# EryiXie/PlaneRecNet

Hardware: AMD Instinct MI355X
Metric: img/s fwd+bwd @480×640 ResNet101-DCN, 1/2/4/8 MI355X + roofline % (higher is better)
Workload: dtype f32 (tensors and accumulation fp32; plain GEMMs and the tap-walked 4x4/s2, 1x1/s2 and sub-pixel convolutions >= 300 tiles: 2xfp16-piece split MFMA, fp32 accumulate; fp32-only rate in fp32_only_run)

## Files before the change

### include/prn.h

```cpp
#ifndef PRN_H
#define PRN_H
#include <stdint.h>
#ifdef __cplusplus
extern "C" {
#endif

#define PRN_BN_SPLITS 32

int prn_version(void);
const char* prn_last_error(void);

enum { PRN_IN_ZERO = 0, PRN_IN_REFLECT = 1, PRN_IN_UP2_REFLECT = 2, PRN_IN_DILATED = 3, PRN_IN_UP2_PHASE = 4,
       PRN_IN_EMBED1 = 5  };
enum { PRN_EPI_NONE = 0, PRN_EPI_RELU = 1, PRN_EPI_SIGMOID = 2 };

enum { PRN_SPLIT_OFF = 0, PRN_SPLIT_PLAN = 1, PRN_SPLIT_ALWAYS = 2 };
enum { PRN_PIECES_BF16 = 0, PRN_PIECES_F16 = 16 };
typedef struct prn_gemm_opts {
  int32_t split_mode;
  int32_t split_kind;
  int32_t split_products;
  int32_t split_min_tiles;
  float split_min_gflop;
  int32_t wgrad_wgs;
  int32_t wgrad_target;
  int32_t wgrad_split;
} prn_gemm_opts;
void prn_gemm_opts_default(prn_gemm_opts* o);

typedef struct prn_conv_desc {
  int32_t B, C, H, W;
  int32_t M;
  int32_t KH, KW;
  int32_t stride, pad;
  int32_t Ho, Wo;
  int32_t in_mode;
  int32_t dil;
  int32_t epilogue;
  int32_t ystride;
  int32_t yH, yW;
  int32_t reserved;
  prn_gemm_opts opts;
} prn_conv_desc;

int64_t prn_conv2d_fwd_ws_bytes(const prn_conv_desc* d);
int prn_conv2d_kernel_kind(const prn_conv_desc* d);
int prn_conv2d_fwd_partials(const prn_conv_desc* d, int64_t* offset_bytes);
int prn_gemm_pipe(int M, int K, int B, int HW, int nz, const prn_gemm_opts* opts);
int64_t prn_split_images_bytes(int M, int K, int nz);
int prn_split_prepare(const float* w, void* images, int M, int K, int nz, int kind, void* stream);
int prn_split_prepare_batched(const void* items_dev, int n_items, int64_t total_blocks, int64_t total_row_blocks, int kind, void* stream);
int prn_conv2d_fwd(const prn_conv_desc* d, const float* x, const float* w, const float* bias,
                   const float* addend, float* y, void* ws, void* stream);
#define PRN_TILE_COUNTERS 4096
int prn_conv2d_fwd_counted(const prn_conv_desc* d, const float* x, const float* w, const void* w_images, const float* bias, const float* addend, float* y,
                           void* ws, unsigned* counters, void* stream, int phase);
#define PRN_MAX_SEGMENTS 6
typedef struct prn_ragged {
  int32_t nseg;
  int32_t H[PRN_MAX_SEGMENTS], W[PRN_MAX_SEGMENTS];
} prn_ragged;
int prn_conv2d_fwd_ragged(const prn_conv_desc* d, const prn_ragged* rg, const float* x, const float* w, const float* bias,
                          const float* addend, float* y, void* stream);
int64_t prn_conv2d_wgrad_ragged_ws_bytes(const prn_conv_desc* d, const prn_ragged* rg);
int prn_conv2d_wgrad_ragged(const prn_conv_desc* d, const prn_ragged* rg, const float* x, const float* dy, float* dw, void* ws,
                            void* stream);

int prn_conv2d_fwd_phase(const prn_conv_desc* d, const float* x, const float* w, const float* bias,
                         const float* addend, float* y, void* ws, void* stream, int phase);

int prn_weight_flip_transpose(const float* w, float* wt, int M, int C, int KH, int KW, void* stream);

typedef struct prn_flip_item {
  const float* src;
  float* dst;
  int M, C, KH, KW;
  int64_t first;
} prn_flip_item;
int prn_weight_flip_transpose_batched(const prn_flip_item* items_dev, int n_items, int64_t total_blocks, void* stream);

int64_t prn_winograd_tiles(int B, int H, int W);
typedef struct prn_winograd_item {
  const float* src;
  float* u;
  float* ut;
  int M, C;
  int64_t first;
} prn_winograd_item;
int prn_winograd_weights_batched(const prn_winograd_item* items_dev, int n_items, int64_t total_blocks, void* stream);
int prn_winograd_input(const float* x, float* V, int B, int C, int H, int W, int in_mode, void* stream);
int64_t prn_gemm_batched_ws_bytes(int M, int C, int P, int nb, const prn_gemm_opts* opts);
int prn_gemm_batched(int M, int C, int P, int nb, const float* U, const void* u_images, const float* V, float* Y, void* ws, const prn_gemm_opts* opts,
                     void* stream);
int prn_winograd_output(const float* Y, const float* bias, const float* addend, float* y, int B, int M, int H, int W, int epilogue, void* stream);
int prn_winograd_output_bn_fwd(const float* Yt, float* x_out, float* stats, const float* gamma, const float* beta, float* y, float* running_mean,
                               float* running_var, int B, int M, int H, int W, float eps, float momentum, int relu, void* stream);
int prn_winograd_output_bn_bwd(const float* Yt, const float* x, const float* stats, const float* gamma, const float* beta, float* dx, float* dgamma,
                               float* dbeta, int B, int M, int H, int W, int relu, void* stream);
int64_t prn_winograd_wgrad_ws_bytes(int B, int C, int H, int W, int M, const prn_gemm_opts* opts);
int prn_winograd_dy(const float* dy, float* Y, int B, int M, int H, int W, void* stream);
int prn_gemm_batched_nt_splits(int M, int C, int P, int nb, const prn_gemm_opts* opts);
int prn_gemm_batched_nt_kind(int M, int C, int P, int nb, const prn_gemm_opts* opts);
int prn_gemm_batched_nt(int M, int C, int P, int nb, const float* A, const float* Bm, float* ws, const prn_gemm_opts* opts, void* stream);
int prn_winograd_dw(const float* partials, float* dw, int M, int C, int splits, void* stream);
int prn_conv3x3_winograd_wgrad(const float* x, const float* dy, float* dw, void* ws, int B, int C, int H, int W, int M, int in_mode, const prn_gemm_opts* opts,
                               void* stream, int phase);
int prn_conv3x3_winograd_wgrad_v(const float* V, const float* dy, float* dw, void* ws, int B, int C, int H, int W, int M, const prn_gemm_opts* opts, void* stream);
int64_t prn_winograd_tiles_ragged(const prn_ragged* rg, int B);
int64_t prn_conv3x3_winograd_ragged_ws_bytes(const prn_ragged* rg, int B, int C, int M, const prn_gemm_opts* opts);
int prn_conv3x3_winograd_ragged(const float* x, const float* U, const void* u_images, const float* bias, const float* addend, float* y, void* ws,
                                const prn_ragged* rg, int B, int C, int M, int epilogue, const prn_gemm_opts* opts, void* stream);
int64_t prn_winograd_wgrad_ragged_ws_bytes(const prn_ragged* rg, int B, int C, int M, const prn_gemm_opts* opts);
int prn_conv3x3_winograd_wgrad_ragged(const float* x, const float* dy, float* dw, void* ws, const prn_ragged* rg, int B, int C, int M, const prn_gemm_opts* opts,
                                      void* stream);
int64_t prn_conv3x3_winograd_ws_bytes(int B, int C, int H, int W, int M, const prn_gemm_opts* opts);
int prn_conv3x3_winograd(const float* x, const float* U, const void* u_images, const float* bias, const float* addend, float* y, void* ws, int B, int C, int H,
                         int W, int M, int in_mode, int epilogue, const prn_gemm_opts* opts, void* stream);

int64_t prn_conv2d_wgrad_ws_bytes(const prn_conv_desc* d);
int prn_conv2d_wgrad_kernel_kind(const prn_conv_desc* d, int G);
int prn_conv2d_wgrad(const prn_conv_desc* d, const float* x, const float* dy, float* dw, void* ws, void* stream);
#define PRN_WGRAD_GROUP_MAX 16
int64_t prn_conv2d_wgrad_grouped_ws_bytes(const prn_conv_desc* d, int G);
int prn_conv2d_wgrad_grouped(const prn_conv_desc* d, int G, const float* const* x, const float* const* dy, float* dw, void* ws, void* stream);
int prn_conv2d_wgrad_phase(const prn_conv_desc* d, const float* x, const float* dy, float* dw, void* ws, void* stream, int phase);

int prn_up2_phase_weights(const float* w, float* wp, int M, int C, void* stream);
int prn_up2_dgrad_weights(const float* w, float* kd, int M, int C, void* stream);
int prn_replicate_fold(const float* dp, float* dx, int B, int C, int H, int W, void* stream);
int prn_space_to_depth2(const float* in, float* out, int B, int C, int H, int W, void* stream);
int prn_up2_wgrad_combine(const float* dwp, float* dw, int M, int C, void* stream);

int prn_pad_fold(const float* dp, float* dx, int B, int C, int H, int W, int up2, void* stream);
// ... 233 lines not shown
```

### planerecnet_amd/_lib.py

```python
import ctypes
import os

_HERE = os.path.dirname(os.path.abspath(__file__))
LIB_PATH = os.environ.get("PRN_LIB") or os.path.join(_HERE, "libprn_hip.so")

c_int, c_float, c_void_p, c_i64 = ctypes.c_int, ctypes.c_float, ctypes.c_void_p, ctypes.c_int64


class GemmOpts(ctypes.Structure):
    _fields_ = [("split_mode", ctypes.c_int32), ("split_kind", ctypes.c_int32), ("split_products", ctypes.c_int32), ("split_min_tiles", ctypes.c_int32),
                ("split_min_gflop", ctypes.c_float), ("wgrad_wgs", ctypes.c_int32), ("wgrad_target", ctypes.c_int32), ("wgrad_split", ctypes.c_int32)]

    def key(self):
        return (self.split_mode, self.split_kind, self.split_products, self.split_min_tiles, self.split_min_gflop, self.wgrad_wgs, self.wgrad_target, self.wgrad_split)


SPLIT_OFF, SPLIT_PLAN, SPLIT_ALWAYS = 0, 1, 2
PIECES_BF16, PIECES_F16 = 0, 16


class ConvDesc(ctypes.Structure):
    _fields_ = [(n, ctypes.c_int32) for n in
                ("B", "C", "H", "W", "M", "KH", "KW", "stride", "pad", "Ho", "Wo", "in_mode", "dil", "epilogue", "ystride", "yH", "yW", "reserved")] + [
                    ("opts", GemmOpts)]


class Ragged(ctypes.Structure):
    _fields_ = [("nseg", ctypes.c_int32), ("H", ctypes.c_int32 * 6), ("W", ctypes.c_int32 * 6)]


class DcnDesc(ctypes.Structure):
    _fields_ = [(n, ctypes.c_int32) for n in ("B", "C", "H", "W", "M", "stride", "pad", "Ho", "Wo", "raw")] + [("max_offset", ctypes.c_float),
                                                                                                              ("epilogue", ctypes.c_int32),
                                                                                                              ("opts", GemmOpts)]


class BottleneckDesc(ctypes.Structure):
    _fields_ = [(n, ctypes.c_int32) for n in ("B", "C", "H", "W", "planes", "stride", "dcn", "downsample", "flags")] + [
        ("eps", ctypes.c_float * 4), ("momentum", ctypes.c_float * 4), ("max_offset", ctypes.c_float), ("reserved", ctypes.c_int32), ("opts", GemmOpts)]


class BottleneckParams(ctypes.Structure):
    _fields_ = [(n, ctypes.c_void_p) for n in (
        "w1", "w2", "w3", "wd", "b2", "w1_img", "w3_img", "wd_img", "u2", "u2_img", "w1_t", "w2_t", "w3_t", "wd_t", "w1_t_img", "w3_t_img", "wd_t_img", "ut2", "ut2_img",
        "w27", "b27", "w27_t", "w2_cols_t", "w2_cols_t_img")] + [(n, ctypes.c_void_p * 4) for n in ("gamma", "beta", "running_mean", "running_var")]


IN_ZERO, IN_REFLECT, IN_UP2_REFLECT, IN_DILATED, IN_UP2_PHASE, IN_EMBED1 = 0, 1, 2, 3, 4, 5
EPI_NONE, EPI_RELU, EPI_SIGMOID = 0, 1, 2
BN_SPLITS = 32

P = c_void_p
_DP = ctypes.POINTER(ConvDesc)
_OP = ctypes.POINTER(GemmOpts)
SIGNATURES = {
    "prn_version": (c_int, []),
    "prn_last_error": (ctypes.c_char_p, []),
    "prn_conv2d_fwd_ws_bytes": (c_i64, [_DP]),
    "prn_conv2d_kernel_kind": (c_int, [_DP]),
    "prn_conv2d_fwd_partials": (c_int, [_DP, ctypes.POINTER(c_i64)]),
    "prn_gemm_opts_default": (None, [_OP]),
    "prn_gemm_pipe": (c_int, [c_int, c_int, c_int, c_int, c_int, _OP]),
    "prn_split_images_bytes": (c_i64, [c_int, c_int, c_int]),
    "prn_split_prepare": (c_int, [P, P, c_int, c_int, c_int, c_int, P]),
    "prn_split_prepare_batched": (c_int, [P, c_int, c_i64, c_i64, c_int, P]),
    "prn_conv2d_fwd": (c_int, [_DP, P, P, P, P, P, P, P]),
    "prn_conv2d_fwd_ragged": (c_int, [_DP, P, P, P, P, P, P, P]),
    "prn_conv2d_wgrad_ragged_ws_bytes": (c_i64, [_DP, P]),
    "prn_conv2d_wgrad_ragged": (c_int, [_DP, P, P, P, P, P, P]),
    "prn_gn_relu_fwd_ragged": (c_int, [P, P, P, P, P, c_int, c_int, c_int, P, c_int, c_float, P]),
    "prn_gn_relu_bwd_ragged": (c_int, [P, P, P, P, P, P, P, P, c_int, c_int, c_int, P, c_int, P]),
    "prn_conv2d_fwd_phase": (c_int, [_DP, P, P, P, P, P, P, P, c_int]),
    "prn_conv2d_fwd_counted": (c_int, [_DP, P, P, P, P, P, P, P, P, P, c_int]),
    "prn_conv2d_wgrad_phase": (c_int, [_DP, P, P, P, P, P, c_int]),
    "prn_weight_flip_transpose": (c_int, [P, P, c_int, c_int, c_int, c_int, P]),
    "prn_weight_flip_transpose_batched": (c_int, [P, c_int, c_i64, P]),
    "prn_winograd_tiles": (c_i64, [c_int, c_int, c_int]),
    "prn_winograd_weights_batched": (c_int, [P, c_int, c_i64, P]),
    "prn_winograd_input": (c_int, [P, P, c_int, c_int, c_int, c_int, c_int, P]),
    "prn_gemm_batched_ws_bytes": (c_i64, [c_int, c_int, c_int, c_int, _OP]),
    "prn_gemm_batched": (c_int, [c_int, c_int, c_int, c_int, P, P, P, P, P, _OP, P]),
    "prn_winograd_output": (c_int, [P, P, P, P, c_int, c_int, c_int, c_int, c_int, P]),
    "prn_winograd_output_bn_fwd": (c_int, [P] * 8 + [c_int] * 4 + [c_float, c_float, c_int, P]),
    "prn_winograd_output_bn_bwd": (c_int, [P] * 8 + [c_int] * 5 + [P]),
    "prn_winograd_wgrad_ws_bytes": (c_i64, [c_int] * 5 + [_OP]),
    "prn_winograd_dy": (c_int, [P, P, c_int, c_int, c_int, c_int, P]),
    "prn_gemm_batched_nt_splits": (c_int, [c_int] * 4 + [_OP]),
    "prn_gemm_batched_nt_kind": (c_int, [c_int] * 4 + [_OP]),
    "prn_conv2d_wgrad_kernel_kind": (c_int, [_DP, c_int]),
    "prn_gemm_batched_nt": (c_int, [c_int, c_int, c_int, c_int, P, P, P, _OP, P]),
    "prn_winograd_dw": (c_int, [P, P, c_int, c_int, c_int, P]),
    "prn_conv3x3_winograd_wgrad": (c_int, [P, P, P, P, c_int, c_int, c_int, c_int, c_int, c_int, _OP, P, c_int]),
    "prn_winograd_tiles_ragged": (c_i64, [P, c_int]),
    "prn_conv3x3_winograd_ragged_ws_bytes": (c_i64, [P, c_int, c_int, c_int, _OP]),
    "prn_conv3x3_winograd_ragged": (c_int, [P, P, P, P, P, P, P, P, c_int, c_int, c_int, c_int, _OP, P]),
    "prn_winograd_wgrad_ragged_ws_bytes": (c_i64, [P, c_int, c_int, c_int, _OP]),
    "prn_conv3x3_winograd_wgrad_ragged": (c_int, [P, P, P, P, P, c_int, c_int, c_int, _OP, P]),
    "prn_conv3x3_winograd_wgrad_v": (c_int, [P, P, P, P, c_int, c_int, c_int, c_int, c_int, _OP, P]),
    "prn_conv3x3_winograd_ws_bytes": (c_i64, [c_int] * 5 + [_OP]),
    "prn_conv3x3_winograd": (c_int, [P, P, P, P, P, P, P, c_int, c_int, c_int, c_int, c_int, c_int, c_int, _OP, P]),
    "prn_conv2d_wgrad_ws_bytes": (c_i64, [_DP]),
    "prn_conv2d_wgrad_grouped_ws_bytes": (c_i64, [_DP, c_int]),
    "prn_conv2d_wgrad_grouped": (c_int, [_DP, c_int, P, P, P, P, P]),
    "prn_conv2d_wgrad": (c_int, [_DP, P, P, P, P, P]),
    "prn_pad_fold": (c_int, [P, P, c_int, c_int, c_int, c_int, c_int, P]),
    "prn_pad_fold_pitched": (c_int, [P, P, c_int, c_int, c_int, c_int, c_int, P]),
    "prn_up2_phase_weights": (c_int, [P, P, c_int, c_int, P]),
    "prn_up2_dgrad_weights": (c_int, [P, P, c_int, c_int, P]),
    "prn_up2_wgrad_combine": (c_int, [P, P, c_int, c_int, P]),
    "prn_space_to_depth2": (c_int, [P, P, c_int, c_int, c_int, c_int, P]),
    "prn_replicate_fold": (c_int, [P, P, c_int, c_int, c_int, c_int, P]),
    "prn_channel_sum": (c_int, [P, P, P, c_int, c_int, c_int, P]),
    "prn_dcn_sample": (c_int, [P, P, P] + [c_int] * 7 + [c_float, P]),
    "prn_dcn_sample_bwd_ws_bytes": (c_i64, [c_int] * 6),
    "prn_dcn_sample_bwd": (c_int, [P, P, P, P, P, P] + [c_int] * 7 + [c_float, P]),
    "prn_dcnv2_table_bytes": (c_i64, [P]),
    "prn_dcnv2_table": (c_int, [P, P, P, P, P]),
    "prn_dcnv2_fwd_ws_bytes": (c_i64, [P]),
    "prn_dcnv2_fwd": (c_int, [P] * 8),
    "prn_dcnv2_fwd_phase": (c_int, [P] * 8 + [c_int]),
    "prn_dcnv2_bwd_weight_ws_bytes": (c_i64, [P]),
    "prn_dcnv2_bwd_weight": (c_int, [P] * 7),
    "prn_dcnv2_bwd_weight_phase": (c_int, [P] * 7 + [c_int]),
    "prn_dcnv2_bwd_ws_bytes": (c_i64, [P]),
    "prn_dcnv2_bwd_input": (c_int, [P] * 9),
    "prn_dcnv2_bwd_input_phase": (c_int, [P] * 9 + [c_int]),
    "prn_bn_kernel_kind": (c_int, [c_int, c_int]),
    "prn_dcnv2_bwd_offset_mask": (c_int, [P] * 8),
    "prn_plane_prior_ws_bytes": (c_i64, [c_int] * 6 + [_OP]),
    "prn_plane_prior_fwd": (c_int, [P] * 7 + [c_int] * 6 + [_OP, P]),
    "prn_plane_prior_fwd_phase": (c_int, [P] * 7 + [c_int] * 6 + [_OP, P, c_int]),
    "prn_plane_prior_wgrad_ws_bytes": (c_i64, [c_int] * 5 + [_OP]),
    "prn_plane_prior_wgrad": (c_int, [P] * 4 + [c_int] * 5 + [_OP, P]),
    "prn_fpn_level_ws_bytes": (c_i64, [c_int] * 8 + [_OP]),
    "prn_fpn_level_fwd": (c_int, [P, P, P, P, c_int, c_int, P, P, P, P, P, P] + [c_int] * 6 + [_OP, P]),
    "prn_frame_to_input": (c_int, [P] + [c_int] * 6 + [P, P, c_int, P, P, P]),
    "prn_mask_loss_ws_floats": (c_int, [c_int]),
    "prn_mask_loss_fwd": (c_int, [P] * 9 + [c_int, c_int, c_int, c_float, c_float, P]),
    "prn_mask_loss_bwd": (c_int, [P] * 8 + [c_int, c_int, P]),
    "prn_vnl_triplets": (c_int, [P] * 12 + [c_int, c_int, c_int, c_float, P]),
    "prn_vnl_scatter": (c_int, [P] * 5 + [c_int, c_int, P]),
    "prn_depth_metrics_ws_doubles": (c_int, []),
    "prn_depth_metrics": (c_int, [P, P, P, P, c_i64, c_float, c_float, P]),
    "prn_vnl_trim_key": (c_int, [P, P, P, P, c_int, P]),
    "prn_vnl_trim_fwd": (c_int, [P, P, P, P, P, P, P, c_int, c_int, c_int, P, P, P, P, P, P]),
    "prn_vnl_trim_ws_bytes": (c_i64, [c_int]),
    "prn_vnl_trim_bwd": (c_int, [P, P, P, P, P, P, P, c_int, c_int, P, P]),
# ... 83 lines not shown
```

### planerecnet_amd/blocks.py

```python
import ctypes
import os
import sys

import torch

from . import _lib, ops, profiling
from ._lib import lib, check

ENABLED = os.environ.get("PRN_BLOCKS", "1") == "1"
HANDOVER = os.environ.get("PRN_BLOCK_HANDOVER", "1") == "1"
SCATTER_ACCUMULATE = os.environ.get("PRN_SCATTER_ACC", "1") == "1"
STATS = {"fwd": 0, "bwd": 0, "resolved": 0, "vouched": 0, "scatter_acc": 0}

BLK_WINOGRAD, BLK_HANDOVER, BLK_KEEP_V, BLK_SCATTER_ACC = 1, 2, 4, 8
CONV2_DIRECT, CONV2_WINOGRAD, CONV2_DCN = 0, 1, 2
(I_SAVE, I_GSAVE, I_FWD_WS, I_BWD_WS, I_HO, I_WO, I_CONV2, I_KEEPS_V, I_A1, I_V, I_A2, I_OM, I_TABLE, I_D1, I_D2, I_D3, I_DD, I_DOM, I_BN_FLOATS, I_HANDOVERS,
 I_W1_IMG, I_W3_IMG, I_WD_IMG, I_W1T_IMG, I_W3T_IMG, I_WDT_IMG, I_U_IMG, I_COLT_IMG, INFO_COUNT) = range(29)

_SCRATCH = {}
_F32 = torch.float32
_empty = torch.empty


def scratch(nbytes, dev):
# ... 68 lines not shown
    if blk.downsample is not None:
        ps += [blk.downsample[0].weight, blk.downsample[1].weight, blk.downsample[1].bias]
    return tuple(ps)


def _state(blk, x, key):
    from .dcn import DeformableConv2d
    oe = ops._opts_entry()
    B, C, H, W = x.shape
    dcn = isinstance(blk.conv2, DeformableConv2d)
    bns = (blk.bn1, blk.bn2, blk.bn3) + ((blk.downsample[1],) if blk.downsample is not None else ())
    eps = [float(m.eps) for m in bns] + [0.0] * (4 - len(bns))
    mom = [float(m.momentum) for m in bns] + [0.0] * (4 - len(bns))
    P = blk.conv1.weight.shape[0]
    d = _lib.BottleneckDesc(B, C, H, W, P, blk.stride, int(dcn), int(blk.downsample is not None), key[2], (ctypes.c_float * 4)(*eps), (ctypes.c_float * 4)(*mom),
                            max(H, W) / 4.0 if dcn else 0.0, 0, oe[0])
    st = _State()
    st.plan = ctypes.create_string_buffer(int(lib.prn_bottleneck_plan_bytes()) + 64)
    st.plan_ref = (ctypes.addressof(st.plan) + 63) & ~63
    check(lib.prn_bottleneck_plan(ctypes.byref(d), st.plan_ref), "prn_bottleneck_plan")
    info = (ctypes.c_int64 * INFO_COUNT)()
    check(lib.prn_bottleneck_plan_info(st.plan_ref, info, INFO_COUNT), "prn_bottleneck_plan_info")
    st.info = info = list(info)
    st.params = _lib.BottleneckParams()
    st.params_ref = ctypes.byref(st.params)
    st.wver, st.epoch, st.keep, st.batched = None, -1, None, False
    st.Ho, st.Wo, st.conv2 = info[I_HO], info[I_WO], info[I_CONV2]
    st.out_shape = (B, 4 * P, st.Ho, st.Wo)
    st.dims = (B, C, H, W, P)
    st.stride, st.dcn, st.ds = blk.stride, dcn, blk.downsample is not None
    st.bn_sizes = [P, P, P, P, 4 * P, 4 * P] + ([4 * P, 4 * P] if st.ds else [])
    st.hb = bool(st.ds and blk.stride == 2)
    st.wino_wgrad = bool(st.conv2 == CONV2_WINOGRAD and ops.WINOGRAD_WGRAD)
    st.max_offset = max(H, W) / 4.0
    st.save_n, st.gsave_n, st.bn_n, st.fwd_ws, st.bwd_ws = info[I_SAVE] // 4, info[I_GSAVE] // 4, info[I_BN_FLOATS], info[I_FWD_WS], info[I_BWD_WS]
    st.ps = _param_list(blk)
    st.bns = bns
    st.stat_bufs = [t for m in bns for t in (m.running_mean, m.running_var)]
    c2 = blk.conv2
    st.convw = (blk.conv1.weight, blk.conv3.weight) + ((c2.offset_conv.weight, c2.modulator_conv.weight, c2.regular_conv.weight) if dcn else (c2.weight,)) + (
        (blk.downsample[0].weight,) if st.ds else ())
    Ho, Wo, s = st.Ho, st.Wo, blk.stride
    Q = 4 * P
    st.shapes = ((B, P, H, W), (B, P, Ho, Wo), (B, Q, Ho, Wo), (B, 27, Ho, Wo))
    pix = ops.WGRAD_GROUP_PIXELS
    st.g_keys = [("conv", (B, C, H, W), (H, W), P, 1, 1, 0, ops.IN_ZERO) if B * H * W <= pix else None,
                 ("conv", (B, P, H, W), (Ho, Wo), P, 3, s, 1, ops.IN_ZERO) if (st.conv2 == CONV2_DIRECT and B * Ho * Wo <= pix) else None,
                 ("conv", (B, P, Ho, Wo), (Ho, Wo), Q, 1, 1, 0, ops.IN_ZERO) if B * Ho * Wo <= pix else None,
                 ("conv", (B, C, H, W), (Ho, Wo), Q, 1, s, 0, ops.IN_ZERO) if B * Ho * Wo <= pix else None]
    return st


def _resolve(blk, st):
    p, info = st.params, st.info
    B, C, H, W, P = st.dims
    Ho, Wo = st.Ho, st.Wo
    Q = 4 * P
    keep = []
    ptr = ops._ptr
    batched = [True]
    BATCHED = ops.BATCHED

    def derived(t):
        keep.append(t)
        if t.data_ptr() not in BATCHED:
            batched[0] = False
        return t

    def images(t, M, K, nz, cols, want):
        return ops.split_images_ptr(t, M, K, nz, cols) if want else None
    w1, w3 = blk.conv1.weight, blk.conv3.weight
    p.w1, p.w3 = ptr(w1), ptr(w3)
    p.w1_img = images(w1, P, C, 1, (B, H * W), info[I_W1_IMG])
    p.w3_img = images(w3, Q, P, 1, (B, Ho * Wo), info[I_W3_IMG])
    w1t, w3t = derived(ops.flip_transpose(w1)), derived(ops.flip_transpose(w3))
    p.w1_t, p.w3_t = ptr(w1t), ptr(w3t)
    p.w1_t_img = images(w1t, C, P, 1, (B, H * W), info[I_W1T_IMG])
    p.w3_t_img = images(w3t, P, Q, 1, (B, Ho * Wo), info[I_W3T_IMG])
    p.wd = p.wd_t = p.wd_img = p.wd_t_img = None
    if st.ds:
        wd = blk.downsample[0].weight
        wdt = derived(ops.flip_transpose(wd))
        p.wd, p.wd_t = ptr(wd), ptr(wdt)
        p.wd_img = images(wd, Q, C, 1, (B, Ho * Wo), info[I_WD_IMG])
        p.wd_t_img = images(wdt, C, Q, 1, (B, H * W), info[I_WDT_IMG])
    p.w2 = p.b2 = p.w2_t = p.u2 = p.ut2 = p.u2_img = p.ut2_img = p.w27 = p.b27 = p.w27_t = p.w2_cols_t = p.w2_cols_t_img = None
    if st.conv2 == CONV2_DCN:
        c2 = blk.conv2
        w27, b27 = c2._merged()
        w2 = c2.regular_conv.weight
        w27t = derived(ops.flip_transpose(w27))
        colt = derived(ops.flip_transpose(w2.view(P, P * 9, 1, 1)))
        p.w2, p.b2 = ptr(w2), ptr(c2.regular_conv.bias)
        p.w27, p.b27, p.w27_t, p.w2_cols_t = ptr(w27), ptr(b27), ptr(w27t), ptr(colt)
        p.w2_cols_t_img = images(colt, 9 * P, P, 1, (B, Ho * Wo), info[I_COLT_IMG])
        keep += [w27, b27]
    elif st.conv2 == CONV2_WINOGRAD:
        w2 = blk.conv2.weight
        U, Ut = ops.winograd_weights(w2)
        derived(U), derived(Ut)
        P4 = lib.prn_winograd_tiles(B, H, W)
        p.u2, p.ut2 = ptr(U), ptr(Ut)
        p.u2_img, p.ut2_img = images(U, P, P, 36, (1, P4), info[I_U_IMG]), images(Ut, P, P, 36, (1, P4), info[I_U_IMG])
        p.w2 = ptr(w2)
    else:
        w2 = blk.conv2.weight
        p.w2, p.w2_t = ptr(w2), ptr(derived(ops.flip_transpose(w2)))
    for i, m in enumerate(st.bns):
        p.gamma[i], p.beta[i], p.running_mean[i], p.running_var[i] = ptr(m.weight), ptr(m.bias), ptr(m.running_mean), ptr(m.running_var)
    st.keep, st.batched = keep, batched[0]
    STATS["resolved"] += 1


class _BottleneckFn(torch.autograd.Function):
    @staticmethod
    def forward(ctx, x, blk, st, hand_back, *ps):
        x0 = x
        if not x.is_contiguous():
            x = x.contiguous()
        dev = x.device
        vs = [w._version for w in st.convw]
        epoch = ops.OPERAND_EPOCH[0]
        if vs != st.wver or st.epoch != epoch:
            R = ops.REFRESHED
            if st.batched and st.epoch == epoch and all([R.get(id(w)) == v for w, v in zip(st.convw, vs)]):
                STATS["vouched"] += 1
            else:
                _resolve(blk, st)
                st.epoch = ops.OPERAND_EPOCH[0]
            st.wver = vs
        y = _empty(st.out_shape, device=dev, dtype=_F32)
        save = _empty(st.save_n, device=dev, dtype=_F32)
        ws = scratch(st.fwd_ws, dev)
        rc = lib.prn_bottleneck_train_fwd(st.plan_ref, st.params_ref, x.data_ptr(), y.data_ptr(), save.data_ptr(), ws.data_ptr(), ops._raw_stream(dev.index))
        if rc:
            check(rc, "prn_bottleneck_train_fwd")
        torch._C._increment_version(st.stat_bufs)
        for m in st.bns:
            ops._count_batch(m)
        ctx.save_for_backward(x, y, save)
        ctx.st, ctx.keep, ctx.vs = st, st.keep, vs
        STATS["fwd"] += 1
        if hand_back:
            ctx.set_materialize_grads(False)
            return y, x0
        return y

    @staticmethod
    def backward(ctx, dy, dfork=None):
        x, y, save = ctx.saved_tensors
        st = ctx.st
        ps = st.ps
        if dy is None:
            return (dfork,) + (None,) * (3 + len(ps))
        if [w._version for w in st.convw] != ctx.vs:
            raise RuntimeError("a parameter of a Bottleneck block was modified between its forward and its backward pass")
        dev = x.device
        if not dy.is_contiguous():
            dy = dy.contiguous()
        info = st.info
        acc = 0
        if dfork is not None and st.hb and SCATTER_ACCUMULATE and dfork.is_contiguous() and dfork._base is None and dfork.shape == x.shape \
                and dfork.dtype == _F32 and dfork._use_count() <= _OWNED[0] and sys.getrefcount(dfork) <= _OWNED[1]:
            dx, acc, dfork = dfork, 1, None
            STATS["scatter_acc"] += 1
        else:
            dx = torch.empty_like(x)
# ... 131 lines not shown
```

### planerecnet_amd/csrc/prn_bottleneck.hip

```cpp
#include "prn_common.h"
#include <string.h>

namespace {

constexpr int32_t PLAN_MAGIC = 0x424c4b36;
constexpr int64_t WINOGRAD_MIN_TILES = 128;

inline int64_t up256(int64_t v) { return (v + 255) & ~255LL; }

struct Plan {
  int32_t magic, pad_;
  prn_bottleneck_desc d;
  int32_t Ho, Wo, P4, conv2_path;
  int32_t small1, small2;
  int32_t lazy1, parts1;
  int32_t v1, lazy2, keep_v;
  int32_t lazy3g, parts3g;
  int32_t v2g, lazy2g;
  int32_t pad2_;
  int64_t parts1_off, parts3g_off;
  prn_conv_desc c1, c2, c3, cd, c27, g1, g2, g3, gd, g27;
  prn_dcn_desc dcn;
  int64_t s_c1, s_a1, s_v, s_c2, s_a2, s_c3, s_cd, s_om, s_table, s_stats[4], save_bytes;
  int64_t q_d3, q_dd, q_d2, q_d1, q_dom, q_bn, gsave_bytes;
// ... 74 lines not shown
#define PRN_WS(expr_, name_) const int64_t name_ = (expr_); if (name_ < 0) return 2
  PRN_WS(prn_conv2d_fwd_ws_bytes(&L.c1), w_c1);
  PRN_WS(prn_conv2d_fwd_ws_bytes(&L.c3), w_c3);
  PRN_WS(d.downsample ? prn_conv2d_fwd_ws_bytes(&L.cd) : 0, w_cd);
  PRN_WS(L.conv2_path == PRN_BLK_CONV2_DIRECT ? prn_conv2d_fwd_ws_bytes(&L.c2) : 0, w_c2);
  PRN_WS(d.dcn ? prn_conv2d_fwd_ws_bytes(&L.c27) : 0, w_c27);
  PRN_WS(d.dcn ? prn_dcnv2_fwd_ws_bytes(&L.dcn) : 0, w_dcnf);
  PRN_WS(d.dcn ? prn_dcnv2_table_bytes(&L.dcn) : 0, n_table);
  PRN_WS(d.dcn ? prn_dcnv2_bwd_ws_bytes(&L.dcn) : 0, w_dcnb);
  PRN_WS(wino ? prn_gemm_batched_ws_bytes(P, P, L.P4, 36, &o) : 0, w_gemm);
  PRN_WS(prn_conv2d_fwd_ws_bytes(&L.g3), w_g3);
  PRN_WS(prn_conv2d_fwd_ws_bytes(&L.g1), w_g1);
  PRN_WS(L.conv2_path == PRN_BLK_CONV2_DIRECT ? prn_conv2d_fwd_ws_bytes(&L.g2) : 0, w_g2);
  PRN_WS(d.dcn ? prn_conv2d_fwd_ws_bytes(&L.g27) : 0, w_g27);
  PRN_WS(d.downsample ? prn_conv2d_fwd_ws_bytes(&L.gd) : 0, w_gd);
#undef PRN_WS
  int64_t at = 0;
  auto put = [&at](int64_t& slot, int64_t bytes) { slot = at; at += up256(bytes); };
  put(L.s_c1, n1); put(L.s_a1, n1);
  put(L.s_v, L.keep_v ? nv : 0);
  put(L.s_c2, n2); put(L.s_a2, n2); put(L.s_c3, n3);
  put(L.s_cd, d.downsample ? n3 : 0);
  put(L.s_om, d.dcn ? nom : 0); put(L.s_table, n_table);
  put(L.s_stats[0], 8LL * P); put(L.s_stats[1], 8LL * P); put(L.s_stats[2], 8LL * Q); put(L.s_stats[3], d.downsample ? 8LL * Q : 0);
  L.save_bytes = at;
  at = 0;
  put(L.q_d3, n3); put(L.q_dd, d.downsample ? n3 : 0); put(L.q_d2, n2); put(L.q_d1, n1); put(L.q_dom, d.dcn ? nom : 0);
  L.q_bn = 2 * P + 2 * P + 2 * Q + (d.downsample ? 2 * Q : 0);
  L.gsave_bytes = at;
  at = 0;
  put(L.f_c1, w_c1); put(L.f_bn, bnws);
  put(L.f_v, (wino && !L.keep_v) ? nv : 0); put(L.f_yt, nv); put(L.f_gemm, w_gemm);
  put(L.f_c2, w_c2); put(L.f_c27, w_c27); put(L.f_dcn, w_dcnf); put(L.f_c3, w_c3); put(L.f_cd, w_cd);
  put(L.f_res, d.downsample ? n3 : 0);
  L.fwd_ws_bytes = at;
  at = 0;
  put(L.b_bn, bnws); put(L.b_dres, n3);
  put(L.b_g3, n2); put(L.b_g3ws, w_g3);
  put(L.b_v, nv); put(L.b_yt, nv); put(L.b_gemm, w_gemm);
  put(L.b_g2, n1); put(L.b_g2ws, w_g2);
  put(L.b_dcn, w_dcnb); put(L.b_dx1, d.dcn ? n1 : 0); put(L.b_g27ws, w_g27);
  put(L.b_g1ws, w_g1);
  put(L.b_gdtmp, d.downsample ? nx : 0); put(L.b_gdws, w_gd);
  L.bwd_ws_bytes = at;
  return 0;
}

const Plan* plan_of(const void* plan, const char* who) {
  const Plan* L = (const Plan*)plan;
  if (L == nullptr || L->magic != PLAN_MAGIC) { prn_set_error("%s: not a plan filled by prn_bottleneck_plan", who); return nullptr; }
  return L;
}

inline float* f32(void* base, int64_t off) { return (float*)((char*)base + off); }
inline void* raw(void* base, int64_t off, int64_t used = 1) { return used ? (void*)((char*)base + off) : nullptr; }

#define PRN_TRY(call_) do { if (int e_ = (call_)) return e_; } while (0)

}

extern "C" int64_t prn_bottleneck_plan_bytes(void) { return (int64_t)sizeof(Plan); }
extern "C" int64_t prn_bottleneck_params_bytes(void) { return (int64_t)sizeof(prn_bottleneck_params); }

extern "C" int prn_bottleneck_plan(const prn_bottleneck_desc* d, void* plan) {
  PRN_REQUIRE(plan != nullptr, "prn_bottleneck_plan: null plan buffer (prn_bottleneck_plan_bytes() bytes, caller-owned)");
  Plan L;
  if (int e = make_plan(d, L)) { memset(plan, 0, sizeof(int32_t)); return e; }
  memcpy(plan, &L, sizeof(L));
  return 0;
}

extern "C" int prn_bottleneck_plan_info(const void* plan, int64_t* out, int n) {
  const Plan* L = plan_of(plan, "prn_bottleneck_plan_info");
  if (!L) return 2;
  PRN_REQUIRE(out != nullptr && n >= PRN_BLK_INFO_COUNT, "prn_bottleneck_plan_info: out must hold PRN_BLK_INFO_COUNT (%d) values", PRN_BLK_INFO_COUNT);
  out[PRN_BLK_SAVE_BYTES] = L->save_bytes; out[PRN_BLK_GSAVE_BYTES] = L->gsave_bytes;
  out[PRN_BLK_FWD_WS_BYTES] = L->fwd_ws_bytes; out[PRN_BLK_BWD_WS_BYTES] = L->bwd_ws_bytes;
  out[PRN_BLK_HO] = L->Ho; out[PRN_BLK_WO] = L->Wo; out[PRN_BLK_CONV2_PATH] = L->conv2_path; out[PRN_BLK_KEEPS_V] = L->keep_v;
  out[PRN_BLK_OFF_A1] = L->s_a1; out[PRN_BLK_OFF_V] = L->s_v; out[PRN_BLK_OFF_A2] = L->s_a2; out[PRN_BLK_OFF_OM] = L->s_om; out[PRN_BLK_OFF_TABLE] = L->s_table;
  out[PRN_BLK_OFF_D1] = L->q_d1; out[PRN_BLK_OFF_D2] = L->q_d2; out[PRN_BLK_OFF_D3] = L->q_d3; out[PRN_BLK_OFF_DD] = L->q_dd; out[PRN_BLK_OFF_DOM] = L->q_dom;
  out[PRN_BLK_BN_GRAD_FLOATS] = L->q_bn;
  out[PRN_BLK_HANDOVERS] = L->lazy1 | (L->v1 << 1) | (L->lazy2 << 2) | (L->lazy3g << 3) | (L->v2g << 4) | (L->lazy2g << 5);
  out[PRN_BLK_NEEDS_W1_IMG] = prn_conv2d_kernel_kind(&L->c1) >= 2; out[PRN_BLK_NEEDS_W3_IMG] = prn_conv2d_kernel_kind(&L->c3) >= 2;
  out[PRN_BLK_NEEDS_WD_IMG] = (L->d.downsample && L->d.stride == 1 && prn_conv2d_kernel_kind(&L->cd) >= 2) ? 1 : 0;
  out[PRN_BLK_NEEDS_W1T_IMG] = prn_conv2d_kernel_kind(&L->g1) >= 2; out[PRN_BLK_NEEDS_W3T_IMG] = prn_conv2d_kernel_kind(&L->g3) >= 2;
  out[PRN_BLK_NEEDS_WDT_IMG] = (L->d.downsample && L->d.stride == 1 && prn_conv2d_kernel_kind(&L->gd) >= 2) ? 1 : 0;
  out[PRN_BLK_NEEDS_U_IMG] = (L->conv2_path == PRN_BLK_CONV2_WINOGRAD && prn_gemm_pipe(L->d.planes, L->d.planes, 1, L->P4, 36, &L->d.opts) >= 1) ? 1 : 0;
  out[PRN_BLK_NEEDS_COLT_IMG] = (L->d.dcn && prn_gemm_pipe(9 * L->d.planes, L->d.planes, L->d.B, L->Ho * L->Wo, 1, &L->d.opts) >= 1) ? 1 : 0;
  return 0;
}

extern "C" int prn_bottleneck_train_fwd(const void* plan, const prn_bottleneck_params* p, const float* x, float* y, void* save, void* ws, void* stream) {
  const Plan* Lp = plan_of(plan, "prn_bottleneck_train_fwd");
  if (!Lp) return 2;
  const Plan& L = *Lp;
  const prn_bottleneck_desc& d = L.d;
  PRN_REQUIRE(p && x && y && save && (ws || L.fwd_ws_bytes == 0), "prn_bottleneck_train_fwd: null tensor / buffer");
  PRN_REQUIRE(p->w1 && p->w3 && (p->w2 || L.conv2_path == PRN_BLK_CONV2_WINOGRAD) && (p->u2 || L.conv2_path != PRN_BLK_CONV2_WINOGRAD) && (!d.downsample || p->wd),
              "prn_bottleneck_train_fwd: a weight operand the plan reads is null");
  PRN_REQUIRE(!d.dcn || (p->w27 && p->b27), "prn_bottleneck_train_fwd: the deformable variant needs the merged offset | modulator weights");
  for (int i = 0; i < (d.downsample ? 4 : 3); ++i)
    PRN_REQUIRE(p->gamma[i] && p->beta[i] && p->running_mean[i] && p->running_var[i], "prn_bottleneck_train_fwd: null BatchNorm parameter (layer %d)", i);
  PRN_REQUIRE(((reinterpret_cast<uintptr_t>(save) | reinterpret_cast<uintptr_t>(ws)) & 255) == 0, "prn_bottleneck_train_fwd: save / ws must be 256-byte aligned");
  const int B = d.B, H = d.H, W = d.W, P = d.planes, Q = 4 * P, Ho = L.Ho, Wo = L.Wo;
  float* c1 = f32(save, L.s_c1); float* a1 = f32(save, L.s_a1); float* c2 = f32(save, L.s_c2); float* a2 = f32(save, L.s_a2); float* c3 = f32(save, L.s_c3);
  float* st1 = f32(save, L.s_stats[0]); float* st2 = f32(save, L.s_stats[1]); float* st3 = f32(save, L.s_stats[2]); float* std_ = f32(save, L.s_stats[3]);
  double* bnws = (double*)raw(ws, L.f_bn);
  const int64_t n1 = (int64_t)B * P * H * W;
  const prn_gemm_opts* o = &d.opts;
  PRN_TRY(prn_conv2d_fwd_counted(&L.c1, x, p->w1, p->w1_img, nullptr, nullptr, c1, raw(ws, L.f_c1, L.f_bn - L.f_c1), nullptr, stream, L.lazy1 ? 1 : 0));
  float* V = L.conv2_path == PRN_BLK_CONV2_WINOGRAD ? (L.keep_v ? f32(save, L.s_v) : f32(ws, L.f_v)) : nullptr;
  const float* in1 = L.lazy1 ? f32(ws, L.f_c1 + L.parts1_off) : c1;
  if (L.v1)
    PRN_TRY(prn_bn_train_fwd_winograd(in1, L.lazy1 ? L.parts1 : 1, L.lazy1 ? n1 : 0, L.lazy1 ? c1 : nullptr, st1, p->gamma[0], p->beta[0], nullptr, a1, p->running_mean[0],
                                      p->running_var[0], V, B, P, H, W, d.eps[0], d.momentum[0], 1, stream));
  else if (L.lazy1)
    PRN_TRY(prn_bn_train_fwd_partials(in1, L.parts1, n1, c1, st1, p->gamma[0], p->beta[0], nullptr, a1, p->running_mean[0], p->running_var[0], B, P, H * W, d.eps[0],
                                      d.momentum[0], 1, stream));
  else
    PRN_TRY(prn_bn_train_fwd(c1, st1, p->gamma[0], p->beta[0], nullptr, a1, p->running_mean[0], p->running_var[0], L.small1 ? nullptr : bnws, B, P, H * W, d.eps[0],
                             d.momentum[0], 1, stream));
  float* Yt = f32(ws, L.f_yt);
  if (L.conv2_path == PRN_BLK_CONV2_WINOGRAD) {
    if (!L.v1) PRN_TRY(prn_winograd_input(a1, V, B, P, H, W, PRN_IN_ZERO, stream));
    PRN_TRY(prn_gemm_batched(P, P, L.P4, 36, p->u2, p->u2_img, V, Yt, raw(ws, L.f_gemm, L.f_c2 - L.f_gemm), o, stream));
    if (!L.lazy2) PRN_TRY(prn_winograd_output(Yt, nullptr, nullptr, c2, B, P, H, W, PRN_EPI_NONE, stream));
  } else if (L.conv2_path == PRN_BLK_CONV2_DCN) {
    float* om = f32(save, L.s_om);
    void* table = raw(save, L.s_table);
    PRN_TRY(prn_conv2d_fwd_counted(&L.c27, a1, p->w27, nullptr, p->b27, nullptr, om, raw(ws, L.f_c27, L.f_dcn - L.f_c27), nullptr, stream, 0));
    PRN_TRY(prn_dcnv2_table(&L.dcn, om, nullptr, table, stream));
    PRN_TRY(prn_dcnv2_fwd(&L.dcn, a1, table, p->w2, p->b2, c2, raw(ws, L.f_dcn, L.f_c3 - L.f_dcn), stream));
  } else {
    PRN_TRY(prn_conv2d_fwd_counted(&L.c2, a1, p->w2, nullptr, nullptr, nullptr, c2, raw(ws, L.f_c2, L.f_c27 - L.f_c2), nullptr, stream, 0));
  }
  if (L.conv2_path == PRN_BLK_CONV2_WINOGRAD && L.lazy2)
    PRN_TRY(prn_winograd_output_bn_fwd(Yt, c2, st2, p->gamma[1], p->beta[1], a2, p->running_mean[1], p->running_var[1], B, P, Ho, Wo, d.eps[1], d.momentum[1], 1, stream));
  else
    PRN_TRY(prn_bn_train_fwd(c2, st2, p->gamma[1], p->beta[1], nullptr, a2, p->running_mean[1], p->running_var[1], L.small2 ? nullptr : bnws, B, P, Ho * Wo, d.eps[1],
                             d.momentum[1], 1, stream));
  PRN_TRY(prn_conv2d_fwd_counted(&L.c3, a2, p->w3, p->w3_img, nullptr, nullptr, c3, raw(ws, L.f_c3, L.f_cd - L.f_c3), nullptr, stream, 0));
  const float* res = x;
  if (d.downsample) {
    float* cd = f32(save, L.s_cd);
    float* rd = f32(ws, L.f_res);
    PRN_TRY(prn_conv2d_fwd_counted(&L.cd, x, p->wd, d.stride == 1 ? p->wd_img : nullptr, nullptr, nullptr, cd, raw(ws, L.f_cd, L.f_res - L.f_cd), nullptr, stream, 0));
    PRN_TRY(prn_bn_train_fwd(cd, std_, p->gamma[3], p->beta[3], nullptr, rd, p->running_mean[3], p->running_var[3], L.small2 ? nullptr : bnws, B, Q, Ho * Wo, d.eps[3],
                             d.momentum[3], 0, stream));
    res = rd;
  }
  return prn_bn_train_fwd(c3, st3, p->gamma[2], p->beta[2], res, y, p->running_mean[2], p->running_var[2], L.small2 ? nullptr : bnws, B, Q, Ho * Wo, d.eps[2], d.momentum[2],
                          1, stream);
}

extern "C" int prn_bottleneck_train_bwd(const void* plan, const prn_bottleneck_params* p, const float* x, const float* y, const float* dy, float* dx,
                                        int dx_accumulate, const void* save_, void* gsave, float* bn_grads, void* ws, void* stream) {
  const Plan* Lp = plan_of(plan, "prn_bottleneck_train_bwd");
  if (!Lp) return 2;
  const Plan& L = *Lp;
  const prn_bottleneck_desc& d = L.d;
  PRN_REQUIRE(p && x && y && dy && dx && save_ && gsave && bn_grads && ws, "prn_bottleneck_train_bwd: null tensor / buffer");
  PRN_REQUIRE(p->w1_t && p->w3_t && (!d.downsample || p->wd_t), "prn_bottleneck_train_bwd: an input-gradient weight layout the plan reads is null");
  PRN_REQUIRE(L.conv2_path != PRN_BLK_CONV2_WINOGRAD || p->ut2, "prn_bottleneck_train_bwd: conv2's Winograd-domain input-gradient operand is null");
  PRN_REQUIRE(L.conv2_path != PRN_BLK_CONV2_DIRECT || p->w2_t, "prn_bottleneck_train_bwd: conv2's input-gradient layout is null");
  PRN_REQUIRE(!d.dcn || (p->w27_t && p->w2_cols_t), "prn_bottleneck_train_bwd: the deformable variant needs the input-gradient layouts of both convolutions");
  PRN_REQUIRE(!dx_accumulate || (d.downsample && d.stride == 2 && (d.flags & PRN_BLK_SCATTER_ACC)),
              "prn_bottleneck_train_bwd: dx_accumulate only for stride-2 downsample blocks planned with PRN_BLK_SCATTER_ACC");
  PRN_REQUIRE(((reinterpret_cast<uintptr_t>(save_) | reinterpret_cast<uintptr_t>(gsave) | reinterpret_cast<uintptr_t>(ws)) & 255) == 0,
              "prn_bottleneck_train_bwd: save / gsave / ws must be 256-byte aligned");
  void* save = const_cast<void*>(save_);
  const int B = d.B, C = d.C, H = d.H, W = d.W, P = d.planes, Q = 4 * P, Ho = L.Ho, Wo = L.Wo;
  const float* c1 = f32(save, L.s_c1); const float* a1 = f32(save, L.s_a1); const float* c2 = f32(save, L.s_c2); const float* c3 = f32(save, L.s_c3);
  const float* st1 = f32(save, L.s_stats[0]); const float* st2 = f32(save, L.s_stats[1]); const float* st3 = f32(save, L.s_stats[2]); const float* std_ = f32(save, L.s_stats[3]);
  float* d3 = f32(gsave, L.q_d3); float* d2 = f32(gsave, L.q_d2); float* d1 = f32(gsave, L.q_d1);
  float* dg1 = bn_grads; float* db1 = dg1 + P; float* dg2 = db1 + P; float* db2 = dg2 + P; float* dg3 = db2 + P; float* db3 = dg3 + Q; float* dgd = db3 + Q; float* dbd = dgd + Q;
  double* bnws = (double*)raw(ws, L.b_bn);
  float* dres = f32(ws, L.b_dres);
  const prn_gemm_opts* o = &d.opts;
  hipStream_t st = (hipStream_t)stream;
  PRN_TRY(prn_bn_bwd(dy, c3, y, st3, p->gamma[2], p->beta[2], d3, dres, dg3, db3, L.small2 ? nullptr : bnws, B, Q, Ho * Wo, 1, 0, stream));
  const float* addx = dres;
  if (d.downsample) {
    float* dd = f32(gsave, L.q_dd);
    PRN_TRY(prn_bn_bwd(dres, f32(save, L.s_cd), nullptr, std_, p->gamma[3], p->beta[3], dd, nullptr, dgd, dbd, L.small2 ? nullptr : bnws, B, Q, Ho * Wo, 0, 0, stream));
    void* gws = raw(ws, L.b_gdws, L.bwd_ws_bytes - L.b_gdws);
    if (d.stride == 1) {
      float* tmp = f32(ws, L.b_gdtmp);
      PRN_TRY(prn_conv2d_fwd_counted(&L.gd, dd, p->wd_t, p->wd_t_img, nullptr, nullptr, tmp, gws, nullptr, stream, 0));
      addx = tmp;
    } else if (dx_accumulate) {
      PRN_TRY(prn_conv2d_fwd_counted(&L.gd, dd, p->wd_t, nullptr, nullptr, dx, dx, gws, nullptr, stream, 0));
      addx = dx;
    } else {
      float* tmp = f32(ws, L.b_gdtmp);
      const hipError_t e = hipMemsetAsync(tmp, 0, (size_t)B * C * H * W * 4, st);
      PRN_REQUIRE(e == hipSuccess, "prn_bottleneck_train_bwd: clearing the strided input gradient failed: %s", hipGetErrorString(e));
      PRN_TRY(prn_conv2d_fwd_counted(&L.gd, dd, p->wd_t, nullptr, nullptr, nullptr, tmp, gws, nullptr, stream, 0));
      addx = tmp;
    }
  }
  float* g3 = f32(ws, L.b_g3);
  PRN_TRY(prn_conv2d_fwd_counted(&L.g3, d3, p->w3_t, p->w3_t_img, nullptr, nullptr, g3, raw(ws, L.b_g3ws, L.b_v - L.b_g3ws), nullptr, stream, L.lazy3g ? 1 : 0));
  const float* in2 = L.lazy3g ? f32(ws, L.b_g3ws + L.parts3g_off) : g3;
  const int64_t n2 = (int64_t)B * P * Ho * Wo;
  float* Vg = f32(ws, L.b_v);
  if (L.v2g)
    PRN_TRY(prn_bn_bwd_winograd(in2, L.lazy3g ? L.parts3g : 1, L.lazy3g ? n2 : 0, c2, nullptr, st2, p->gamma[1], p->beta[1], d2, nullptr, dg2, db2, Vg, B, P, Ho, Wo, 1, 0, stream));
  else if (L.lazy3g)
    PRN_TRY(prn_bn_bwd_partials(in2, L.parts3g, n2, c2, nullptr, st2, p->gamma[1], p->beta[1], d2, nullptr, dg2, db2, B, P, Ho * Wo, 1, 0, stream));
  else
    PRN_TRY(prn_bn_bwd(g3, c2, nullptr, st2, p->gamma[1], p->beta[1], d2, nullptr, dg2, db2, L.small2 ? nullptr : bnws, B, P, Ho * Wo, 1, 0, stream));
  float* g2 = f32(ws, L.b_g2);
  float* Ytg = f32(ws, L.b_yt);
  if (L.conv2_path == PRN_BLK_CONV2_WINOGRAD) {
    if (!L.v2g) PRN_TRY(prn_winograd_input(d2, Vg, B, P, H, W, PRN_IN_ZERO, stream));
    PRN_TRY(prn_gemm_batched(P, P, L.P4, 36, p->ut2, p->ut2_img, Vg, Ytg, raw(ws, L.b_gemm, L.b_g2 - L.b_gemm), o, stream));
    if (!L.lazy2g) PRN_TRY(prn_winograd_output(Ytg, nullptr, nullptr, g2, B, P, H, W, PRN_EPI_NONE, stream));
  } else if (L.conv2_path == PRN_BLK_CONV2_DCN) {
    const float* om = f32(save, L.s_om);
    float* dom = f32(gsave, L.q_dom);
    float* dx1 = f32(ws, L.b_dx1);
    void* cws = raw(ws, L.b_dcn);
    PRN_TRY(prn_dcnv2_bwd_input(&L.dcn, d2, p->w2_cols_t, p->w2_cols_t_img, om, nullptr, dx1, cws, stream));
    PRN_TRY(prn_dcnv2_bwd_offset_mask(&L.dcn, a1, om, nullptr, dom, nullptr, cws, stream));
    PRN_TRY(prn_conv2d_fwd_counted(&L.g27, dom, p->w27_t, nullptr, nullptr, dx1, g2, raw(ws, L.b_g27ws, L.b_g1ws - L.b_g27ws), nullptr, stream, 0));
  } else {
    PRN_TRY(prn_conv2d_fwd_counted(&L.g2, d2, p->w2_t, nullptr, nullptr, nullptr, g2, raw(ws, L.b_g2ws, L.b_dcn - L.b_g2ws), nullptr, stream, 0));
  }
  if (L.conv2_path == PRN_BLK_CONV2_WINOGRAD && L.lazy2g)
// ... 6 lines not shown
```

### planerecnet_amd/csrc/prn_common.h

```cpp
#pragma once
#include <hip/hip_runtime.h>
#include <stdint.h>
#include <stdio.h>
#include "../../include/prn.h"

#define PRN_WAVE 64

void prn_set_error(const char* fmt, ...);

#include <stdlib.h>
static inline int prn_env_int(const char* name, int dflt) {
  const char* e = getenv(name);
  return e ? atoi(e) : dflt;
}
struct prn_env4 { int v[4]; };
static inline prn_env4 prn_env_ints(const char* name) {
  prn_env4 r = {{0, 0, 0, 0}};
  if (const char* e = getenv(name)) sscanf(e, "%d,%d,%d,%d", &r.v[0], &r.v[1], &r.v[2], &r.v[3]);
  return r;
}

extern int prn_skip_mask;
#define PRN_SKIPPED(bit) (__builtin_expect(prn_skip_mask & (bit), 0))
#define PRN_REPS(bit) (__builtin_expect(prn_skip_mask & ((bit) | ((bit) << 8)), 0) ? ((prn_skip_mask & (bit)) ? 0 : 2) : 1)
// ... 16 lines not shown
  } while (0)

__device__ __forceinline__ int prn_xcd_remap(int bid, int nblocks) {
  const int per = nblocks >> 3;
  if (per == 0 || bid >= (per << 3)) return bid;
  return (bid & 7) * per + (bid >> 3);
}

__device__ __forceinline__ void prn_idx3(int64_t i, int W, int H, int& x, int& y, int64_t& z) {
  if (i < (1LL << 31)) {
    const unsigned u = (unsigned)i, q = u / (unsigned)W, q2 = q / (unsigned)H;
    x = (int)(u - q * (unsigned)W); y = (int)(q - q2 * (unsigned)H); z = q2;
  } else {
    x = (int)(i % W); y = (int)((i / W) % H); z = i / ((int64_t)W * H);
  }
}

struct __attribute__((packed, aligned(4))) prn_f4u { float v[4]; };
constexpr int PRN_EPT = 4;
__host__ __device__ inline unsigned prn_ept_blocks(int64_t n) { return (unsigned)((((n + PRN_EPT - 1) / PRN_EPT) + 255) / 256); }
#define PRN_EPT_BEGIN(total_) \
  const int64_t T_ = (int64_t)gridDim.x * 256, i0_ = (int64_t)blockIdx.x * 256 + threadIdx.x; \
  float v_[PRN_EPT]; \
  _Pragma("unroll") for (int k_ = 0; k_ < PRN_EPT; ++k_) { \
    const int64_t i = (i0_ + k_ * T_ < (total_)) ? i0_ + k_ * T_ : (total_) - 1;
#define PRN_EPT_END(total_, out_) \
  } \
  _Pragma("unroll") for (int k_ = 0; k_ < PRN_EPT; ++k_) if (i0_ + k_ * T_ < (total_)) (out_)[i0_ + k_ * T_] = v_[k_];


__device__ __forceinline__ float wave_sum(float v) {
#pragma unroll
  for (int o = 32; o > 0; o >>= 1) v += __shfl_xor(v, o, 64);
  return v;
}
__device__ __forceinline__ double wave_sum_d(double v) {
#pragma unroll
  for (int o = 32; o > 0; o >>= 1) v += __shfl_xor(v, o, 64);
  return v;
}

__device__ __forceinline__ void block_sum2(double& a, double& b, double* sm) {
  a = wave_sum_d(a);
  b = wave_sum_d(b);
  const int w = threadIdx.x >> 6, nw = blockDim.x >> 6;
  __syncthreads();
  if ((threadIdx.x & 63) == 0) { sm[w] = a; sm[nw + w] = b; }
  __syncthreads();
  double ra = 0.0, rb = 0.0;
  for (int i = 0; i < nw; ++i) { ra += sm[i]; rb += sm[nw + i]; }
  a = ra; b = rb;
}

__device__ __forceinline__ void bt6(const float* v, float* o) {
  o[0] = 4.f * v[0] - 5.f * v[2] + v[4];
  o[1] = -4.f * (v[1] + v[2]) + v[3] + v[4];
  o[2] = 4.f * (v[1] - v[2]) - v[3] + v[4];
  o[3] = -2.f * v[1] - v[2] + 2.f * v[3] + v[4];
  o[4] = 2.f * v[1] - v[2] - 2.f * v[3] + v[4];
  o[5] = 4.f * v[1] - 5.f * v[3] + v[5];
}
__device__ __forceinline__ void at6(const float* m, float* o) {
  const float s12 = m[1] + m[2], d12 = m[1] - m[2], s34 = m[3] + m[4], d34 = m[3] - m[4];
  o[0] = m[0] + s12 + s34;
  o[1] = d12 + 2.f * d34;
  o[2] = s12 + 4.f * s34;
  o[3] = d12 + 8.f * d34 + m[5];
}

static inline int cdiv(int64_t a, int64_t b) { return (int)((a + b - 1) / b); }

int prn_launch_reduce_epilogue(const float* ws, const float* bias, const float* addend, float* y, int64_t total, int M, int HoWo, int splits,
                               int epi, hipStream_t st);
int prn_launch_reduce_splits(const float* ws, float* out, int64_t n, int splits, hipStream_t st);
int prn_quantise_splits(int64_t tiles, int splits);
int prn_gemm_batched_epi(int M, int C, int P, int nb, const float* U, const void* u_images, const float* V, float* Y, void* ws, const prn_gemm_opts* opts, int epi,
                         void* stream);

int prn_split_gemm_plan(int M, int K, int B, int HW, int nz, const prn_gemm_opts* opts);
int64_t prn_split_gemm_image_bytes(int M, int K, int nz);
int64_t prn_split_gemm_partial_bytes(int M, int B, int HW, int nz, int splits);
int prn_split_gemm(const float* w, const void* w_images, const float* x, const float* bias, const float* addend, float* y, void* images_ws, float* partial, int M,
                   int K, int B, int HW, int nz, int64_t zw, int64_t zx, int64_t zy, int epi, int splits, const prn_gemm_opts* opts, hipStream_t st, int phase);
int prn_split_conv_taps(const float* w, const float* x, const float* bias, const float* addend, float* y, void* images_ws, float* partial, int M, int C, int B, int XH,
                        int XW, int Ho, int Wo, int KH, int KW, int stride, int pad, int epi, int splits, const prn_gemm_opts* o, hipStream_t st, int phase);
int prn_split_conv_up2(const float* wp, const float* x, const float* bias, float* y, void* images_ws, int M, int C, int B, int H, int W, int epi, const prn_gemm_opts* o,
                       hipStream_t st);
static inline prn_gemm_opts prn_opts_or_zero(const prn_gemm_opts* o) {
  prn_gemm_opts z;
  if (o) return *o;
  z.split_mode = 0; z.split_kind = 0; z.split_products = 0; z.split_min_tiles = 0; z.split_min_gflop = 0.f; z.wgrad_wgs = 0; z.wgrad_target = 0; z.wgrad_split = 0;
  return z;
}

int prn_wgrad16_plan(int M, int C, int64_t N, int HW, int nz, const prn_gemm_opts* opts);
int prn_wgrad16_launch(const float* dy, const float* x, const float* const* gdy, const float* const* gx, int ngroup, float* out, int M, int C, int B, int HW, int nz,
                       int64_t zdy, int64_t zx, int splits, const prn_gemm_opts* opts, hipStream_t st);
```

### planerecnet_amd/csrc/prn_conv.hip

```cpp
#include <stddef.h>
#include <stdlib.h>
#include <type_traits>
#include "prn_common.h"

typedef float f32x16 __attribute__((ext_vector_type(16)));

namespace {

constexpr int MAX_SEG = 6;
struct Seg {
  int nseg;
  int n0[MAX_SEG + 1];
  int H[MAX_SEG], W[MAX_SEG];
  int x0[MAX_SEG], y0[MAX_SEG];
};
__device__ __forceinline__ int seg_find(const Seg& g, int n) {
  int s = 0;
#pragma unroll
  for (int t = 1; t < MAX_SEG; ++t)
    if (t < g.nseg && n >= g.n0[t]) s = t;
  return s;
}
template <class Args>
__device__ __forceinline__ int seg_read(size_t member_offset, int s) {
// ... 1438 lines not shown
  return n;
}
int conv_fwd_impl(const prn_conv_desc* d, const prn_ragged* rg, const float* x, const float* w, const float* bias, const float* addend, float* y,
                  void* ws, void* stream, int phase, unsigned* counters = nullptr, const void* w_images = nullptr);
int conv_wgrad_impl(const prn_conv_desc* d, const prn_ragged* rg, const float* x, const float* dy, float* dw, void* ws, void* stream, int phase);
}

extern "C" int prn_conv2d_kernel_kind(const prn_conv_desc* d) {
  if (check_desc(d, "prn_conv2d_kernel_kind")) return -1;
  if (direct_small_m(d) || direct_one_c(d)) return 1;
  int ss = split_plan_of(d);
  if (ss == 0) ss = taps_plan_of(d);
  if (ss == 0) ss = up2_plan_of(d);
  return ss == 0 ? 0 : (ss == 1 ? 2 : 3);
}

extern "C" int prn_conv2d_fwd_partials(const prn_conv_desc* d, int64_t* offset_bytes) {
  if (check_desc(d, "prn_conv2d_fwd_partials")) return -1;
  PRN_REQUIRE(offset_bytes != nullptr, "prn_conv2d_fwd_partials: null offset");
  *offset_bytes = 0;
  if (direct_small_m(d) || direct_one_c(d)) return 0;
  if (const int ss = split_plan_of(d)) {
    *offset_bytes = (prn_split_gemm_image_bytes(d->M, d->C, 1) + 255) & ~255LL;
    return ss > 1 ? ss : 0;
  }
  if (taps_plan_of(d) || up2_plan_of(d)) return 0;
  const Geo g = geo_of(d);
  const FwdPlan p = plan_fwd(d->M, (int64_t)d->B * g.gH * g.gW, d->C * d->KH * d->KW, narrow_available(d->KH, d->in_mode), g.phases, g.nosplit,
                             wide_ks(d->KH, d->in_mode));
  return p.splits > 1 ? p.splits : 0;
}

extern "C" int prn_conv2d_fwd_phase(const prn_conv_desc* d, const float* x, const float* w, const float* bias,
                                    const float* addend, float* y, void* ws, void* stream, int phase) {
  return conv_fwd_impl(d, nullptr, x, w, bias, addend, y, ws, stream, phase);
}

extern "C" int prn_conv2d_fwd_counted(const prn_conv_desc* d, const float* x, const float* w, const void* w_images, const float* bias, const float* addend,
                                      float* y, void* ws, unsigned* counters, void* stream, int phase) {
  return conv_fwd_impl(d, nullptr, x, w, bias, addend, y, ws, stream, phase, counters, w_images);
}

extern "C" int prn_conv2d_fwd_ragged(const prn_conv_desc* d, const prn_ragged* rg, const float* x, const float* w, const float* bias,
                                     const float* addend, float* y, void* stream) {
  PRN_REQUIRE(rg != nullptr, "prn_conv2d_fwd_ragged: null segment list");
  return conv_fwd_impl(d, rg, x, w, bias, addend, y, nullptr, stream, 0);
}

namespace {
int conv_fwd_impl(const prn_conv_desc* d0, const prn_ragged* rg, const float* x, const float* w, const float* bias, const float* addend, float* y,
                  void* ws, void* stream, int phase, unsigned* counters, const void* w_images) {
  prn_conv_desc dd;
  const prn_conv_desc* d = d0;
  if (rg && d0) {
    dd = *d0; dd.H = dd.Ho = rg->H[0]; dd.W = dd.Wo = rg->W[0]; d = &dd;
  }
  if (int e = check_desc(d, "prn_conv2d_fwd")) return e;
  PRN_REQUIRE(x && w && y, "prn_conv2d_fwd: null tensor");
  if (rg == nullptr && (direct_small_m(d) || direct_one_c(d))) {
    if (phase == 2) return 0;
    hipStream_t sd = (hipStream_t)stream;
    if (direct_small_m(d)) {
      const dim3 grid(cdiv((int64_t)d->B * d->H * d->W, 256)), block(256);
#define PRN_SMALL_M(MODE_, MM_) hipLaunchKernelGGL((conv3x3_small_m_kernel<MODE_, MM_>), grid, block, 0, sd, x, w, bias, addend, y, d->B, d->C, d->H, d->W, \
                                                   d->pad, d->epilogue)
      if (d->in_mode == PRN_IN_ZERO) { if (d->M == 1) PRN_SMALL_M(PRN_IN_ZERO, 1); else PRN_SMALL_M(PRN_IN_ZERO, 2); }
      else { if (d->M == 1) PRN_SMALL_M(PRN_IN_REFLECT, 1); else PRN_SMALL_M(PRN_IN_REFLECT, 2); }
#undef PRN_SMALL_M
    } else {
      hipLaunchKernelGGL(conv3x3_one_c_kernel, dim3(cdiv((int64_t)d->B * d->Ho * d->Wo, 256)), dim3(256), 0, sd, x, w, bias, addend, y, d->B, d->H, d->W,
                         d->M, d->pad, d->Ho, d->Wo, d->epilogue);
    }
    PRN_CHECK_LAUNCH("prn_conv2d_fwd/direct");
    return 0;
  }
  if (rg == nullptr && ws != nullptr) {
    if (const int ss = split_plan_of(d)) {
      const int64_t ib = (prn_split_gemm_image_bytes(d->M, d->C, 1) + 255) & ~255LL;
      return prn_split_gemm(w, w_images, x, bias, addend, y, ws, (float*)((char*)ws + ib), d->M, d->C, d->B, d->H * d->W, 1, 0, 0, 0, d->epilogue, ss, &d->opts,
                            (hipStream_t)stream, phase);
    }
    if (up2_plan_of(d) && addend == nullptr && (reinterpret_cast<uintptr_t>(y) & 15) == 0) {
      if (phase == 2) return 0;
      return prn_split_conv_up2(w, x, bias, y, ws, d->M, d->C, d->B, d->H, d->W, d->epilogue, &d->opts, (hipStream_t)stream);
    }
    if (const int st = taps_plan_of(d)) {
      const int64_t ib = (prn_split_gemm_image_bytes(d->M, d->C * d->KH * d->KW, 1) + 255) & ~255LL;
      return prn_split_conv_taps(w, x, bias, addend, y, ws, (float*)((char*)ws + ib), d->M, d->C, d->B, d->H, d->W, d->Ho, d->Wo, d->KH, d->KW, d->stride, d->pad, d->epilogue,
                                 st, &d->opts, (hipStream_t)stream, phase);
    }
  }
  ConvArgs a;
  a.x = x; a.w = w; a.bias = bias; a.addend = addend; a.y = y; a.ws = (float*)ws;
  a.B = d->B; a.C = d->C; a.H = d->H; a.W = d->W; a.M = d->M; a.stride = d->stride; a.pad = d->pad;
  const Geo g = geo_of(d);
  a.Ho = g.gH; a.Wo = g.gW; a.epi = d->epilogue;
  a.K = d->C * d->KH * d->KW; a.N = d->B * g.gH * g.gW; a.HoWo = g.gH * g.gW; a.HW = d->H * d->W;
  a.xbytes = d->B * d->C * d->H * d->W * 4; a.wbytes = d->M * a.K * 4;
  a.ystride = 1; a.yW = g.gW; a.yHW = a.HoWo;
  a.zx = a.zw = a.zy = 0;
  if (g.phases == 4) { a.ystride = 2; a.yW = d->Wo; a.yHW = d->Ho * d->Wo; }
  else if (d->ystride == 2) { a.ystride = 2; a.yW = d->yW; a.yHW = d->yH * d->yW; }
  if (rg) a.N = (int)seg_pixels(rg, d->B);
  FwdPlan p = plan_fwd(a.M, a.N, a.K, narrow_available(d->KH, d->in_mode), g.phases, g.nosplit || rg != nullptr, wide_ks(d->KH, d->in_mode));
  if (rg) {
    int bn = 32 * p.wn * p.tn;
    bool ok = true;
    int64_t n = 0;
    for (int sI = 0; sI < rg->nseg; ++sI) { ok = ok && n % bn == 0; n += (int64_t)d->B * rg->H[sI] * rg->W[sI]; }
    if (!(ok && n % bn == 0) && !(p.tm == 1 && p.tn == 1 && p.wm == 2)) { p.tm = 1; p.tn = 1; p.wm = 2; p.wn = 2; }
    if (int e = fill_seg(a.seg, rg, d, 32 * p.wn * p.tn, "prn_conv2d_fwd_ragged")) return e;
  } else {
    a.seg.nseg = 0;
  }
  PRN_REQUIRE(p.splits == 1 || ws != nullptr, "prn_conv2d_fwd: workspace required (%d K-splits, see prn_conv2d_fwd_ws_bytes)", p.splits);
  hipStream_t st = (hipStream_t)stream;
  const int mode = d->in_mode;
  int tail_pieces = 0;
  const int tail_tiles = (rg == nullptr && ws != nullptr) ? tail_of(d, g, p, &tail_pieces) : 0;
  if (phase == 2) goto reduce_only;
  if (d->KH == 1) {
    PRN_REQUIRE(mode == PRN_IN_ZERO || mode == PRN_IN_DILATED, "prn_conv2d_fwd: 1x1 kernels take zero or dilated input mode");
    if (mode == PRN_IN_ZERO) launch_fwd<1, PRN_IN_ZERO>(a, p, st, 1, tail_tiles, tail_pieces, counters); else launch_fwd<1, PRN_IN_DILATED>(a, p, st, 1, 0, 0, counters);
  } else if (d->KH == 2) {
    launch_fwd<2, PRN_IN_UP2_PHASE>(a, p, st, 4);
  } else if (d->KH == 3) {
    if (mode == PRN_IN_ZERO) launch_fwd<3, PRN_IN_ZERO>(a, p, st, 1, tail_tiles, tail_pieces, counters);
    else if (mode == PRN_IN_REFLECT) launch_fwd<3, PRN_IN_REFLECT>(a, p, st, 1, tail_tiles, tail_pieces, counters);
    else if (mode == PRN_IN_UP2_REFLECT) launch_fwd<3, PRN_IN_UP2_REFLECT>(a, p, st, 1, 0, 0, counters);
    else launch_fwd<3, PRN_IN_DILATED>(a, p, st, 1, 0, 0, counters);
  } else if (d->KH == 4) {
    launch_fwd<4, PRN_IN_ZERO>(a, p, st, 1, 0, 0, counters);
  } else {
    if (mode == PRN_IN_ZERO) launch_fwd<7, PRN_IN_ZERO>(a, p, st, 1, 0, 0, counters); else launch_fwd<7, PRN_IN_DILATED>(a, p, st, 1, 0, 0, counters);
  }
  PRN_CHECK_LAUNCH("prn_conv2d_fwd");
  if (phase == 1) return 0;
reduce_only:
  {
    const bool tail_launch = tail_pieces > 1 && (mode == PRN_IN_ZERO || mode == PRN_IN_REFLECT) && (d->KH == 1 || d->KH == 3);
    if (fused_reduce_ok(a, p, g.phases, tail_launch ? tail_pieces : 0, counters)) return 0;
  }
  if (p.splits > 1) {
    const int64_t total = (int64_t)a.B * a.M * a.HoWo;
    hipLaunchKernelGGL(reduce_epilogue_kernel, dim3(cdiv(total, 1024)), dim3(256), 0, st, (const float*)ws, bias, addend, y, total, a.M, a.HoWo,
                       p.splits, a.epi);
    PRN_CHECK_LAUNCH("prn_conv2d_fwd/reduce");
  } else if (tail_pieces > 1 && (mode == PRN_IN_ZERO || mode == PRN_IN_REFLECT) && (d->KH == 1 || d->KH == 3)) {
    const int64_t total = (int64_t)a.B * a.M * a.HoWo;
    const int bn = 32 * p.wn * p.tn, tilesM = cdiv(a.M, 32 * p.wm * p.tm);
    const int n_start = (int)(((int64_t)tilesM * cdiv(a.N, bn) - tail_tiles) / tilesM) * bn;
    const int ntail4 = (a.N - n_start) / 4;
    hipLaunchKernelGGL(reduce_tail_kernel, dim3(cdiv((int64_t)a.M * ntail4, 256)), dim3(256), 0, st, (const float*)ws, bias, addend, y, total, a.M, a.HoWo,
                       n_start, ntail4, tail_pieces, a.epi);
    PRN_CHECK_LAUNCH("prn_conv2d_fwd/tail reduce");
  }
  return 0;
}
}

extern "C" int64_t prn_conv2d_wgrad_ws_bytes(const prn_conv_desc* d) {
  if (check_desc(d, "prn_conv2d_wgrad_ws_bytes")) return -1;
  const int K = d->C * d->KH * d->KW;
  if (direct_small_m(d)) return (int64_t)direct_wgrad_splits(d) * d->M * K * 4;
  if (const int s16 = wgrad16_plan_of(d, 1)) return s16 > 1 ? (int64_t)s16 * d->M * K * 4 : 0;
  const Geo g = geo_of(d);
  WgPlan p = plan_wgrad(d->opts, d->M, K, (int64_t)d->B * g.gH * g.gW, g.phases);
  return p.splits > 1 ? (int64_t)p.splits * g.phases * d->M * K * 4 : 0;
}

extern "C" int prn_conv2d_wgrad_kernel_kind(const prn_conv_desc* d, int G) {
// ... 294 lines not shown
```

### planerecnet_amd/csrc/prn_gemm_split.hip

```cpp
#include "prn_common.h"
#include <stdlib.h>

namespace {

typedef __attribute__((ext_vector_type(8))) __bf16 bf16x8_t;
typedef __attribute__((ext_vector_type(16))) float f32x16_t;
typedef int i32x4_t __attribute__((ext_vector_type(4)));
typedef float f32x4_t __attribute__((ext_vector_type(4)));

constexpr int BM = 128, BK = 32;
constexpr int IMG_U4 = 1536;

__device__ __forceinline__ void split2(float x0, float x1, unsigned& h, unsigned& m, unsigned& l) {
  const unsigned u0 = __float_as_uint(x0), u1 = __float_as_uint(x1);
  const float r0 = x0 - __uint_as_float(u0 & 0xffff0000u), r1 = x1 - __uint_as_float(u1 & 0xffff0000u);
  const unsigned v0 = __float_as_uint(r0), v1 = __float_as_uint(r1);
  const float s0 = r0 - __uint_as_float(v0 & 0xffff0000u), s1 = r1 - __uint_as_float(v1 & 0xffff0000u);
  h = __builtin_amdgcn_perm(u1, u0, 0x07060302u);
  m = __builtin_amdgcn_perm(v1, v0, 0x07060302u);
  l = __builtin_amdgcn_perm(__float_as_uint(s1), __float_as_uint(s0), 0x07060302u);
}

__global__ void split_prepare_kernel(const float* __restrict__ w, uint4* __restrict__ img, int M, int K, long long zw, int mtiles, int kslices, long long total) {
  const long long i = (long long)blockIdx.x * 256 + threadIdx.x;
// ... 95 lines not shown
  for (int ks = ks0; ks < ks1; ++ks) {
    const int st = (ks - ks0) & 1;
    asm volatile("s_waitcnt vmcnt(0)" ::: "memory");
    __syncthreads();
    const bool more = ks + 1 < ks1;
    const int kn = more ? ks + 1 : ks;
    if (more) SPLIT_DMA(ks + 1, st ^ 1);
    SPLIT_LOADB(kn);
    __builtin_amdgcn_sched_barrier(0);
    SPLIT_STEP(0);
    __builtin_amdgcn_sched_barrier(0);
    SPLIT_STEP(1);
    SPLIT_PIECES();
  }
#undef SPLIT_DMA
#undef SPLIT_LOADB
#undef SPLIT_PIECES
#undef SPLIT_STEP
  const bool cok = px < HW;
  if (a.splits > 1) {
    float* pb = a.partial + (long long)sp * a.slice + ((long long)z * a.B + b) * (long long)M * HW;
#pragma unroll
    for (int i = 0; i < 4; ++i)
#pragma unroll
      for (int e = 0; e < 16; ++e) {
        const int row = mt * BM + i * 32 + gs * 4 + (e >> 2) * 8 + (e & 3);
        if (cok && row < M) pb[(long long)row * HW + px] = __uint_as_float(__float_as_uint(acc[i][e]) ^ sflip32);
      }
    return;
  }
  float* yb = a.y + (long long)z * a.zy + (long long)b * M * HW;
  const float* ab = a.addend ? a.addend + (long long)z * a.zy + (long long)b * M * HW : nullptr;
#pragma unroll
  for (int i = 0; i < 4; ++i) {
    const int rbase = mt * BM + i * 32 + gs * 4;
    float bv[16], av[16];
#pragma unroll
    for (int e = 0; e < 16; ++e) {
      const int row = rbase + (e >> 2) * 8 + (e & 3); const int rc = row < M ? row : M - 1;
      bv[e] = a.bias ? a.bias[rc] : 0.f; av[e] = ab ? ab[(long long)rc * HW + pxc] : 0.f;
    }
#pragma unroll
    for (int e = 0; e < 16; ++e) {
      const int row = rbase + (e >> 2) * 8 + (e & 3);
      float v = __uint_as_float(__float_as_uint(acc[i][e]) ^ sflip32) + bv[e] + av[e];
      if (a.epi == PRN_EPI_RELU) v = fmaxf(v, 0.f);
      else if (a.epi == PRN_EPI_SIGMOID) v = 1.f / (1.f + expf(-v));
      if (cok && row < M) yb[(long long)row * HW + px] = v;
    }
  }
}

typedef __attribute__((ext_vector_type(8))) _Float16 f16x8_t;
typedef __attribute__((ext_vector_type(2))) _Float16 f16x2_t;
typedef float f32x2_t __attribute__((ext_vector_type(2)));
constexpr int IMG16_U4 = 1024;

__device__ __forceinline__ void split2_f16(float x0, float x1, unsigned& h, unsigned& l) {
  f16x2_t hv, lv;
  hv[0] = (_Float16)x0; hv[1] = (_Float16)x1;
  h = __builtin_bit_cast(unsigned, hv);
  float r0, r1;
  asm("v_fma_mix_f32 %0, %1, -1.0, %2 op_sel:[0,0,0] op_sel_hi:[1,0,0]" : "=v"(r0) : "v"(h), "v"(x0));
  asm("v_fma_mix_f32 %0, %1, -1.0, %2 op_sel:[1,0,0] op_sel_hi:[1,0,0]" : "=v"(r1) : "v"(h), "v"(x1));
  lv[0] = (_Float16)r0; lv[1] = (_Float16)r1;
  l = __builtin_bit_cast(unsigned, lv);
}

__global__ __launch_bounds__(256) void split16_rowmax_kernel(const float* __restrict__ w, int* __restrict__ ex, int M, int K, long long zw, int Mpad, long long rows) {
  const long long row = (long long)blockIdx.x * 4 + (threadIdx.x >> 6);
  if (row >= rows) return;
  const int lane = threadIdx.x & 63;
  const long long z = row / Mpad; const int m = (int)(row - z * Mpad);
  float mx = 0.f;
  if (m < M) {
    const float* wr = w + z * zw + (long long)m * K;
    for (int k = lane; k < K; k += 64) mx = fmaxf(mx, fabsf(wr[k]));
  }
#pragma unroll
  for (int o = 32; o > 0; o >>= 1) mx = fmaxf(mx, __shfl_xor(mx, o, 64));
  if (lane == 0) ex[row] = mx > 0.f ? __builtin_amdgcn_frexp_expf(mx) : 0;
}

__global__ void split16_prepare_kernel(const float* __restrict__ w, uint4* __restrict__ img, const int* __restrict__ ex, int M, int K, long long zw, int mtiles, int kslices,
                                       long long total, int taps = 1) {
  const long long i = (long long)blockIdx.x * 256 + threadIdx.x;
  if (i >= total) return;
  const int g = i % 4; const int r = (i / 4) % 128; const long long t = i / 512;
  const int ks = t % kslices; const long long zm = t / kslices; const int mt = zm % mtiles; const long long z = zm / mtiles;
  const int m = mt * 128 + r, k0 = ks * 32 + g * 8;
  const int sh = 14 - ex[z * (mtiles * 128) + m];
  float v[8];
  const int C = K / taps;
#pragma unroll
  for (int j = 0; j < 8; ++j) {
    const int kp = k0 + j;
    const int ksrc = taps > 1 ? (kp % C) * taps + kp / C : kp;
    v[j] = (m < M && kp < K) ? ldexpf(w[z * zw + (long long)m * K + ksrc], sh) : 0.f;
  }
  uint4 h, l;
  split2_f16(v[0], v[1], h.x, l.x); split2_f16(v[2], v[3], h.y, l.y); split2_f16(v[4], v[5], h.z, l.z); split2_f16(v[6], v[7], h.w, l.w);
  uint4* o = img + t * IMG16_U4;
  o[g * 128 + r] = h; o[(4 + g) * 128 + r] = l;
}

#ifdef PRN_S16_TIMING
__device__ long long prn_s16_dbg[8192 * 6];
#define S16_T(slot_) do { if (t == 0 && blockIdx.x + gridDim.x * blockIdx.y < 8192) prn_s16_dbg[(blockIdx.x + gridDim.x * blockIdx.y) * 6 + (slot_)] = (long long)wall_clock64(); } while (0)
__device__ long long prn_s16_it[64 * 4 * 4];
#define S16_IT(slot_) do { if (t == 0 && (blockIdx.x == 0 || blockIdx.x == gridDim.x / 2) && blockIdx.y == 0 && ks - ks0 < 64) { \
    if ((slot_) == 2) asm volatile("s_waitcnt vmcnt(0)" ::: "memory"); \
    prn_s16_it[((blockIdx.x ? 1 : 0) * 64 + (ks - ks0)) * 4 + (slot_)] = (long long)wall_clock64(); } } while (0)
extern "C" int prn_debug_s16_iter(long long* host, int n) { return (int)hipMemcpyFromSymbol(host, HIP_SYMBOL(prn_s16_it), sizeof(long long) * (size_t)n); }
extern "C" int prn_debug_s16_timing(long long* host, int n) { return (int)hipMemcpyFromSymbol(host, HIP_SYMBOL(prn_s16_dbg), sizeof(long long) * (size_t)n); }
#else
#define S16_T(slot_) do { } while (0)
#define S16_IT(slot_) do { } while (0)
#endif

__device__ __forceinline__ void store4_policy(float* p, float4 v, int pol) {
  const f32x4_t q = {v.x, v.y, v.z, v.w};
  if (pol == 0) *reinterpret_cast<float4*>(p) = v;
  else if (pol == 1) asm volatile("global_store_dwordx4 %0, %1, off sc1" ::"v"(p), "v"(q) : "memory");
  else if (pol == 2) asm volatile("global_store_dwordx4 %0, %1, off nt" ::"v"(p), "v"(q) : "memory");
  else if (pol == 3) asm volatile("global_store_dwordx4 %0, %1, off sc0 sc1" ::"v"(p), "v"(q) : "memory");
  else asm volatile("global_store_dwordx4 %0, %1, off sc1 nt" ::"v"(p), "v"(q) : "memory");
}

struct Split16Args {
  const uint4* img; const int* ex; const float* x; const float* bias; const float* addend; float* y; float* partial;
  int M, K, B, HW, epi, mtiles, kslices, ptiles, total, splits;
  int wide;
  int store_policy;
  long long zx, zy, slice;
  int C, XH, XW, Wo, KW, stride, pad;
};

template <int NP, int TAPS = 0>
__global__ __launch_bounds__(256) __attribute__((amdgpu_waves_per_eu(3, 3))) void split16_gemm_kernel(const Split16Args a) {
  __shared__ uint4 lds[2 * IMG16_U4];
  const int t = threadIdx.x, lane = t & 63, wave = __builtin_amdgcn_readfirstlane(t >> 6);
  const int id = prn_xcd_remap(blockIdx.x, a.total);
  const int mt = id % a.mtiles; const int rest = id / a.mtiles;
  const int pt = rest % a.ptiles; const int zb = rest / a.ptiles; const int b = zb % a.B, z = zb / a.B;
  const int sp = blockIdx.y;
  const int ks0 = (int)((long long)a.kslices * sp / a.splits), ks1 = (int)((long long)a.kslices * (sp + 1) / a.splits);
  const int HW = a.HW, M = a.M;
  const int r = lane & 31, gs = lane >> 5;
  S16_T(0);
#ifdef PRN_S16_TIMING
  if (t == 0 && blockIdx.x + gridDim.x * blockIdx.y < 8192) {
    unsigned hw, xcc; asm volatile("s_getreg_b32 %0, hwreg(HW_REG_HW_ID)" : "=s"(hw)); asm volatile("s_getreg_b32 %0, hwreg(HW_REG_XCC_ID)" : "=s"(xcc));
    prn_s16_dbg[(blockIdx.x + gridDim.x * blockIdx.y) * 6 + 4] = ((long long)(xcc & 15) << 32) | hw;
  }
#endif
  const int px = pt * 128 + wave * 32 + r;
  const int pxc = px < HW ? px : HW - 1;
  const int XHW = TAPS ? a.XH * a.XW : HW;
  const int XK = TAPS ? a.C : a.K;
  const float* xb = a.x + (long long)z * a.zx + (long long)b * XK * XHW;
  const __amdgpu_buffer_rsrc_t xrs = __builtin_amdgcn_make_buffer_rsrc(const_cast<float*>(xb), 0, XK * XHW * 4, 0x00020000);
  const int xoff = (pxc + gs * 8 * HW) * 4;
  int choff[16];
#pragma unroll
  for (int j = 0; j < 16; ++j) choff[j] = __builtin_amdgcn_readfirstlane(min(((j >> 3) * 16 + (j & 7)) * XHW * 4, XK * XHW * 4));
  const int t_oi = TAPS ? pxc / a.Wo : 0, t_oj = TAPS ? pxc - t_oi * a.Wo : 0;
  const int t_iy0 = t_oi * a.stride - a.pad, t_ix0 = t_oj * a.stride - a.pad;
  auto tap_vo = [&](int ks_) -> int {
    const int k0 = ks_ * BK, tp = __builtin_amdgcn_readfirstlane(k0 / a.C), c0 = __builtin_amdgcn_readfirstlane(k0 - tp * a.C);
    const int ty = __builtin_amdgcn_readfirstlane(tp / a.KW), tx = __builtin_amdgcn_readfirstlane(tp - ty * a.KW);
    int iy = t_iy0 + ty, ix = t_ix0 + tx;
    bool ok = (unsigned)iy < (unsigned)a.XH && (unsigned)ix < (unsigned)a.XW && k0 < a.K;
    if (TAPS == 2) {
      iy = min(max(t_oi + (z >> 1) - 1 + ty, 0), a.XH - 1); ix = min(max(t_oj + (z & 1) - 1 + tx, 0), a.XW - 1);
      ok = k0 < a.K;
    }
    return ok ? (iy * a.XW + ix + (c0 + gs * 8) * XHW) * 4 : (int)0x80000000u;
  };
  const uint4* ag = a.img + ((long long)(z * a.mtiles + mt) * a.kslices) * IMG16_U4;
  const i32x4_t adesc = make_desc(ag, (unsigned)a.kslices * IMG16_U4 * 16u);
  const unsigned lds0 = (unsigned)(unsigned long long)(void*)lds;
  float rn[16];
// ... 95 lines not shown
  float* yb = a.y + (long long)z * a.zy + (long long)b * M * HW;
  const float* ab = a.addend ? a.addend + (long long)z * a.zy + (long long)b * M * HW : nullptr;
  float* pb = a.splits > 1 ? a.partial + (long long)sp * a.slice + ((long long)z * a.B + b) * (long long)M * HW : nullptr;
  if (a.wide) {
    __syncthreads();
    float* cw = reinterpret_cast<float*>(lds) + wave * (32 * 36);
    int* exl = reinterpret_cast<int*>(lds) + 4 * (32 * 36);
    if (t < 128) exl[t] = exm[t];
    __syncthreads();
    const int crow = lane >> 3, ccol = (lane & 7) * 4;
    const int px4 = pt * 128 + wave * 32 + ccol;
    const bool pok = px4 < HW;
    const bool fin = a.splits == 1;
#pragma unroll
    for (int i = 0; i < 4; ++i) {
#pragma unroll
      for (int e = 0; e < 16; ++e) {
        const int ro = (e >> 2) * 8 + (e & 3) + gs * 4;
        cw[ro * 36 + r] = __uint_as_float(__float_as_uint(ldexpf(acc[i][e], erun + exl[i * 32 + ro] - 28)) ^ sflip32);
      }
      __builtin_amdgcn_wave_barrier();
#pragma unroll
      for (int q = 0; q < 4; ++q) {
        const int rl = crow + 8 * q, row = mt * BM + i * 32 + rl;
        float4 v = *reinterpret_cast<const float4*>(&cw[rl * 36 + ccol]);
        if (!pok || row >= M) continue;
        const long long idx = (long long)row * HW + px4;
        if (TAPS == 2) {
          if (a.bias) { const float bm = a.bias[row]; v.x += bm; v.y += bm; v.z += bm; v.w += bm; }
          if (a.epi == PRN_EPI_RELU) { v.x = fmaxf(v.x, 0.f); v.y = fmaxf(v.y, 0.f); v.z = fmaxf(v.z, 0.f); v.w = fmaxf(v.w, 0.f); }
          const int oi4 = px4 / a.Wo, oj4 = px4 - oi4 * a.Wo;
          float* yp = a.y + (((long long)b * M + row) * (2 * a.XH) + 2 * oi4 + (z >> 1)) * (2 * a.XW) + 2 * oj4 + (z & 1);
          yp[0] = v.x; yp[2] = v.y; yp[4] = v.z; yp[6] = v.w;
          continue;
        }
        if (fin) {
          if (a.bias) { const float bm = a.bias[row]; v.x += bm; v.y += bm; v.z += bm; v.w += bm; }
          if (ab) { const float4 t4 = *reinterpret_cast<const float4*>(ab + idx); v.x += t4.x; v.y += t4.y; v.z += t4.z; v.w += t4.w; }
          if (a.epi == PRN_EPI_RELU) { v.x = fmaxf(v.x, 0.f); v.y = fmaxf(v.y, 0.f); v.z = fmaxf(v.z, 0.f); v.w = fmaxf(v.w, 0.f); }
          else if (a.epi == PRN_EPI_SIGMOID) { v.x = 1.f / (1.f + expf(-v.x)); v.y = 1.f / (1.f + expf(-v.y)); v.z = 1.f / (1.f + expf(-v.z)); v.w = 1.f / (1.f + expf(-v.w)); }
          store4_policy(yb + idx, v, a.store_policy);
        } else {
          store4_policy(pb + idx, v, a.store_policy);
        }
      }
      __builtin_amdgcn_wave_barrier();
    }
#ifdef PRN_S16_TIMING
    asm volatile("s_waitcnt vmcnt(0)" ::: "memory");
#endif
    S16_T(3);
    return;
  }
  if (a.splits > 1) {
#pragma unroll
    for (int i = 0; i < 4; ++i)
#pragma unroll
      for (int e = 0; e < 16; ++e) {
        const int rl = i * 32 + gs * 4 + (e >> 2) * 8 + (e & 3), row = mt * BM + rl;
        if (cok && row < M) pb[(long long)row * HW + px] = __uint_as_float(__float_as_uint(ldexpf(acc[i][e], erun + exm[rl] - 28)) ^ sflip32);
      }
    return;
  }
#pragma unroll
  for (int i = 0; i < 4; ++i) {
    const int rl0 = i * 32 + gs * 4, rbase = mt * BM + rl0;
    float bv[16], av[16]; int ev[16];
#pragma unroll
    for (int e = 0; e < 16; ++e) {
      const int ro = (e >> 2) * 8 + (e & 3), row = rbase + ro; const int rc = row < M ? row : M - 1;
      bv[e] = a.bias ? a.bias[rc] : 0.f; av[e] = ab ? ab[(long long)rc * HW + pxc] : 0.f; ev[e] = exm[rl0 + ro];
    }
#pragma unroll
    for (int e = 0; e < 16; ++e) {
      const int row = rbase + (e >> 2) * 8 + (e & 3);
      float v = __uint_as_float(__float_as_uint(ldexpf(acc[i][e], erun + ev[e] - 28)) ^ sflip32) + bv[e] + av[e];
      if (a.epi == PRN_EPI_RELU) v = fmaxf(v, 0.f);
      else if (a.epi == PRN_EPI_SIGMOID) v = 1.f / (1.f + expf(-v));
      if (cok && row < M) yb[(long long)row * HW + px] = v;
    }
  }
}

struct PrepItem { const float* src; uint4* dst; int M, K, nz, pad; long long zw; long long first; };
__global__ void split_prepare_batched_kernel(const PrepItem* __restrict__ items, int n) {
  int lo = 0, hi = n - 1;
  const long long blk = blockIdx.x;
  while (lo < hi) { const int mid = (lo + hi + 1) >> 1; if (items[mid].first <= blk) lo = mid; else hi = mid - 1; }
  const PrepItem it = items[lo];
  const int mtiles = (it.M + 127) / 128, kslices = (it.K + 31) / 32;
  const long long total = (long long)it.nz * mtiles * kslices * 512;
  const long long i = (blk - it.first) * 256 + threadIdx.x;
  if (i >= total) return;
  const int g = i % 4; const int r = (i / 4) % 128; const long long t = i / 512;
  const int ks = t % kslices; const long long zm = t / kslices; const int mt = zm % mtiles; const long long z = zm / mtiles;
  const int m = mt * 128 + r, k0 = ks * 32 + g * 8;
  float v[8];
#pragma unroll
  for (int j = 0; j < 8; ++j) v[j] = (m < it.M && k0 + j < it.K) ? it.src[z * (long long)it.M * it.K + (long long)m * it.K + k0 + j] : 0.f;
  uint4 h, mm, l;
  split2(v[0], v[1], h.x, mm.x, l.x); split2(v[2], v[3], h.y, mm.y, l.y); split2(v[4], v[5], h.z, mm.z, l.z); split2(v[6], v[7], h.w, mm.w, l.w);
  uint4* o = it.dst + t * IMG_U4;
  o[(0 * 4 + g) * 128 + r] = h; o[(1 * 4 + g) * 128 + r] = mm; o[(2 * 4 + g) * 128 + r] = l;
}

__device__ __forceinline__ PrepItem find_item(const PrepItem* items, int n, long long blk, bool rows) {
  int lo = 0, hi = n - 1;
  while (lo < hi) { const int mid = (lo + hi + 1) >> 1; if ((rows ? items[mid].zw : items[mid].first) <= blk) lo = mid; else hi = mid - 1; }
  return items[lo];
}
__global__ __launch_bounds__(256) void split16_rowmax_batched_kernel(const PrepItem* __restrict__ items, int n) {
  const PrepItem it = find_item(items, n, blockIdx.x, true);
  const int mtiles = (it.M + 127) / 128, Mpad = mtiles * 128;
  const long long rows = (long long)it.nz * Mpad;
  const long long row = ((long long)blockIdx.x - it.zw) * 4 + (threadIdx.x >> 6);
  if (row >= rows) return;
  const int kslices = (it.K + 31) / 32;
  int* ex = (int*)((char*)it.dst + (long long)it.nz * mtiles * kslices * IMG16_U4 * 16);
  const int lane = threadIdx.x & 63;
  const long long z = row / Mpad; const int m = (int)(row - z * Mpad);
  float mx = 0.f;
  if (m < it.M) {
    const float* wr = it.src + z * (long long)it.M * it.K + (long long)m * it.K;
    if ((it.K & 3) == 0 && (reinterpret_cast<uintptr_t>(it.src) & 15) == 0) {
      const float4* w4 = reinterpret_cast<const float4*>(wr);
      for (int k = lane; k < (it.K >> 2); k += 64) { const float4 q = w4[k]; mx = fmaxf(fmaxf(mx, fmaxf(fabsf(q.x), fabsf(q.y))), fmaxf(fabsf(q.z), fabsf(q.w))); }
    } else {
      for (int k = lane; k < it.K; k += 64) mx = fmaxf(mx, fabsf(wr[k]));
    }
  }
#pragma unroll
  for (int o = 32; o > 0; o >>= 1) mx = fmaxf(mx, __shfl_xor(mx, o, 64));
  if (lane == 0) ex[row] = mx > 0.f ? __builtin_amdgcn_frexp_expf(mx) : 0;
}
__global__ void split16_prepare_batched_kernel(const PrepItem* __restrict__ items, int n) {
  const PrepItem it = find_item(items, n, blockIdx.x, false);
  const int mtiles = (it.M + 127) / 128, kslices = (it.K + 31) / 32;
  const long long total = (long long)it.nz * mtiles * kslices * 512;
  const long long i = ((long long)blockIdx.x - it.first) * 256 + threadIdx.x;
  if (i >= total) return;
  const int* ex = (const int*)((const char*)it.dst + (long long)it.nz * mtiles * kslices * IMG16_U4 * 16);
  const int g = i % 4; const int r = (i / 4) % 128; const long long t = i / 512;
  const int ks = t % kslices; const long long zm = t / kslices; const int mt = zm % mtiles; const long long z = zm / mtiles;
  const int m = mt * 128 + r, k0 = ks * 32 + g * 8;
  const int sh = 14 - ex[z * (mtiles * 128) + m];
  float v[8];
  const float* wr = it.src + z * (long long)it.M * it.K + (long long)m * it.K + k0;
  if (m < it.M && k0 + 8 <= it.K && (it.K & 3) == 0 && (reinterpret_cast<uintptr_t>(it.src) & 15) == 0) {
    const float4 a = *reinterpret_cast<const float4*>(wr), b = *reinterpret_cast<const float4*>(wr + 4);
    v[0] = ldexpf(a.x, sh); v[1] = ldexpf(a.y, sh); v[2] = ldexpf(a.z, sh); v[3] = ldexpf(a.w, sh);
    v[4] = ldexpf(b.x, sh); v[5] = ldexpf(b.y, sh); v[6] = ldexpf(b.z, sh); v[7] = ldexpf(b.w, sh);
  } else {
#pragma unroll
    for (int j = 0; j < 8; ++j) v[j] = (m < it.M && k0 + j < it.K) ? ldexpf(wr[j], sh) : 0.f;
  }
  uint4 h, l;
  split2_f16(v[0], v[1], h.x, l.x); split2_f16(v[2], v[3], h.y, l.y); split2_f16(v[4], v[5], h.z, l.z); split2_f16(v[6], v[7], h.w, l.w);
  uint4* o = it.dst + t * IMG16_U4;
  o[g * 128 + r] = h; o[(4 + g) * 128 + r] = l;
}

}

int prn_split_gemm_plan(int M, int K, int B, int HW, int nz, const prn_gemm_opts* o) {
  if (o == nullptr || o->split_mode == PRN_SPLIT_OFF) return 0;
  if (M <= 0 || K <= 0 || B <= 0 || HW <= 0 || nz <= 0) return 0;
  if ((int64_t)K * HW >= (1LL << 29) || (int64_t)M * HW >= (1LL << 29)) return 0;
  const int mtiles = cdiv(M, 128), kslices = cdiv(K, 32);
  const int64_t tiles = (int64_t)mtiles * cdiv(HW, 128) * B * nz;
  int splits = 1;
  if (tiles < 300) {
    splits = (int)(640 / (tiles > 0 ? tiles : 1));
    if (splits > kslices / 8) splits = kslices / 8;
    static const int smax = prn_env_int("PRN_SPLIT_KSPLIT_MAX", 3);
    const int wide = splits > 4 ? 4 : splits;
    if (splits > smax) splits = smax;
    if (o->split_mode == PRN_SPLIT_PLAN && tiles * splits < o->split_min_tiles && tiles * wide >= o->split_min_tiles) splits = wide;
    if (splits < 1) splits = 1;
  }
  if (o->split_mode == PRN_SPLIT_ALWAYS) return splits;
  if ((int64_t)mtiles * 128 * 4 > (int64_t)M * 5) return 0;
  if (2.0 * M * K * (double)HW * B * nz < (double)o->split_min_gflop * 1e9) return 0;
  if (tiles * splits < o->split_min_tiles) return 0;
  return splits;
}
extern "C" void prn_gemm_opts_default(prn_gemm_opts* o) {
  if (!o) return;
  o->split_mode = PRN_SPLIT_PLAN; o->split_kind = PRN_PIECES_F16; o->split_products = 3; o->split_min_tiles = 300; o->split_min_gflop = 4.0f;
  o->wgrad_wgs = 0; o->wgrad_target = 0; o->wgrad_split = PRN_SPLIT_PLAN;
}
extern "C" int64_t prn_split_images_bytes(int M, int K, int nz) {
  if (M <= 0 || K <= 0 || nz <= 0) return -1;
  return prn_split_gemm_image_bytes(M, K, nz);
}
extern "C" int prn_split_prepare_batched(const void* items_dev, int n_items, int64_t total_blocks, int64_t total_row_blocks, int kind, void* stream) {
  PRN_REQUIRE(items_dev && n_items > 0 && total_blocks > 0 && total_blocks < (1LL << 31), "prn_split_prepare_batched: bad arguments");
  PRN_REQUIRE(kind == PRN_PIECES_F16 || kind == PRN_PIECES_BF16, "prn_split_prepare_batched: kind is PRN_PIECES_F16 or PRN_PIECES_BF16");
  if (kind == PRN_PIECES_F16) {
    PRN_REQUIRE(total_row_blocks > 0 && total_row_blocks < (1LL << 31), "prn_split_prepare_batched: the fp16 piece format needs the row-block count");
    hipLaunchKernelGGL(split16_rowmax_batched_kernel, dim3((unsigned)total_row_blocks), dim3(256), 0, (hipStream_t)stream, (const PrepItem*)items_dev, n_items);
    hipLaunchKernelGGL(split16_prepare_batched_kernel, dim3((unsigned)total_blocks), dim3(256), 0, (hipStream_t)stream, (const PrepItem*)items_dev, n_items);
    PRN_CHECK_LAUNCH("prn_split_prepare_batched/f16");
    return 0;
  }
  hipLaunchKernelGGL(split_prepare_batched_kernel, dim3((unsigned)total_blocks), dim3(256), 0, (hipStream_t)stream, (const PrepItem*)items_dev, n_items);
  PRN_CHECK_LAUNCH("prn_split_prepare_batched");
  return 0;
}
namespace {
int cut_weight(const float* w, void* images, int M, int K, int nz, long long zw, int kind, hipStream_t st, const char* who, int taps = 1) {
  const int mtiles = cdiv(M, 128), kslices = cdiv(K, 32);
  const long long ptotal = (long long)nz * mtiles * kslices * 512;
  if (kind == PRN_PIECES_F16) {
    int* ex = (int*)((char*)images + (int64_t)nz * mtiles * kslices * IMG16_U4 * 16);
    const long long rows = (long long)nz * mtiles * 128;
    hipLaunchKernelGGL(split16_rowmax_kernel, dim3(cdiv(rows, 4)), dim3(256), 0, st, w, ex, M, K, zw, mtiles * 128, rows);
    hipLaunchKernelGGL(split16_prepare_kernel, dim3(cdiv(ptotal, 256)), dim3(256), 0, st, w, (uint4*)images, (const int*)ex, M, K, zw, mtiles, kslices, ptotal, taps);
  } else {
    hipLaunchKernelGGL(split_prepare_kernel, dim3(cdiv(ptotal, 256)), dim3(256), 0, st, w, (uint4*)images, M, K, zw, mtiles, kslices, ptotal);
  }
  PRN_CHECK_LAUNCH(who);
  return 0;
}
}
extern "C" int prn_split_prepare(const float* w, void* images, int M, int K, int nz, int kind, void* stream) {
  PRN_REQUIRE(w && images && M > 0 && K > 0 && nz > 0 && (reinterpret_cast<uintptr_t>(images) & 15) == 0, "prn_split_prepare: bad arguments");
  PRN_REQUIRE(kind == PRN_PIECES_F16 || kind == PRN_PIECES_BF16, "prn_split_prepare: kind is PRN_PIECES_F16 or PRN_PIECES_BF16");
  return cut_weight(w, images, M, K, nz, (long long)M * K, kind, (hipStream_t)stream, "prn_split_prepare");
}
extern "C" int prn_gemm_pipe(int M, int K, int B, int HW, int nz, const prn_gemm_opts* opts) {
  return prn_split_gemm_plan(M, K, B, HW, nz, opts);
}
int64_t prn_split_gemm_image_bytes(int M, int K, int nz) { return (int64_t)nz * cdiv(M, 128) * cdiv(K, 32) * IMG_U4 * 16 + (int64_t)nz * cdiv(M, 128) * 128 * 4; }
int64_t prn_split_gemm_partial_bytes(int M, int B, int HW, int nz, int splits) { return splits > 1 ? (int64_t)splits * nz * B * M * HW * 4 : 0; }

int prn_split_gemm(const float* w, const void* w_images, const float* x, const float* bias, const float* addend, float* y, void* images_ws, float* partial, int M,
                   int K, int B, int HW, int nz, int64_t zw, int64_t zx, int64_t zy, int epi, int splits, const prn_gemm_opts* o, hipStream_t st, int phase) {
  PRN_REQUIRE(o != nullptr && w && x && y && (splits == 1 || partial), "prn_split_gemm: null operand");
  const int mtiles = cdiv(M, 128), kslices = cdiv(K, 32), ptiles = cdiv(HW, 128);
  PRN_REQUIRE((int64_t)kslices * IMG_U4 * 16 < (1LL << 31) && (int64_t)K * HW < (1LL << 29), "prn_split_gemm: operand larger than a buffer descriptor");
  const int kind = o->split_kind;
  PRN_REQUIRE(kind == PRN_PIECES_F16 || kind == PRN_PIECES_BF16, "prn_split_gemm: unknown piece format %d", kind);
  {
    static const int dbg = prn_env_int("PRN_SPLIT_DEBUG", 0);
    if (dbg) fprintf(stderr, "prn_split_gemm M=%d K=%d B=%d HW=%d nz=%d splits=%d epi=%d addend=%d\n", M, K, B, HW, nz, splits, epi, addend != nullptr);
  }
  if (phase != 2) {
    const void* images = w_images;
    if (images == nullptr) {
      PRN_REQUIRE(images_ws != nullptr, "prn_split_gemm: no workspace for the weight images");
      if (int e = cut_weight(w, images_ws, M, K, nz, (long long)zw, kind, st, "prn_split_gemm/prepare")) return e;
      images = images_ws;
    }
    PRN_REQUIRE((reinterpret_cast<uintptr_t>(images) & 15) == 0, "prn_split_gemm: images must be 16-byte aligned");
    if (kind == PRN_PIECES_F16) {
      Split16Args a;
      a.img = (const uint4*)images; a.ex = (const int*)((const char*)images + (int64_t)nz * mtiles * kslices * IMG16_U4 * 16);
      a.x = x; a.bias = bias; a.addend = addend; a.y = y; a.partial = partial;
      a.M = M; a.K = K; a.B = B; a.HW = HW; a.epi = epi; a.mtiles = mtiles; a.kslices = kslices; a.ptiles = ptiles;
      a.total = mtiles * ptiles * B * nz; a.splits = splits; a.zx = zx; a.zy = zy; a.slice = (long long)nz * B * M * HW;
      a.C = K; a.XH = 1; a.XW = HW; a.Wo = HW; a.KW = 1; a.stride = 1; a.pad = 0;
      {
        auto al16 = [](const void* q) { return (reinterpret_cast<uintptr_t>(q) & 15) == 0; };
        static const int wide_on = prn_env_int("PRN_SPLIT_WIDE_STORE", 1);
        a.wide = wide_on && (HW & 3) == 0 && ((int64_t)M * HW & 3) == 0 && (zy & 3) == 0 && al16(y) && al16(addend) && al16(partial);
        static const int policy = prn_env_int("PRN_SPLIT_STORE_POLICY", 1);
        a.store_policy = policy;
      }
      if (o->split_products >= 4) hipLaunchKernelGGL(split16_gemm_kernel<4>, dim3(a.total, splits), dim3(256), 0, st, a);
      else hipLaunchKernelGGL(split16_gemm_kernel<3>, dim3(a.total, splits), dim3(256), 0, st, a);
      PRN_CHECK_LAUNCH("prn_split_gemm/f16");
    } else {
      SplitArgs a;
      a.img = (const uint4*)images; a.x = x; a.bias = bias; a.addend = addend; a.y = y; a.partial = partial;
      a.M = M; a.K = K; a.B = B; a.HW = HW; a.epi = epi; a.mtiles = mtiles; a.kslices = kslices; a.ptiles = ptiles;
      a.total = mtiles * ptiles * B * nz; a.splits = splits; a.zx = zx; a.zy = zy; a.slice = (long long)nz * B * M * HW;
      hipLaunchKernelGGL(split_gemm_kernel, dim3(a.total, splits), dim3(256), 0, st, a);
      PRN_CHECK_LAUNCH("prn_split_gemm");
    }
  }
  if (splits > 1 && phase != 1) {
    PRN_REQUIRE(nz == 1 || (zy == (int64_t)B * M * HW), "prn_split_gemm: K splits need a dense output");
    return prn_launch_reduce_epilogue(partial, bias, addend, y, (int64_t)nz * B * M * HW, M, HW, splits, epi, st);
  }
  return 0;
}

int prn_split_conv_taps(const float* w, const float* x, const float* bias, const float* addend, float* y, void* images_ws, float* partial, int M, int C, int B, int XH,
                        int XW, int Ho, int Wo, int KH, int KW, int stride, int pad, int epi, int splits, const prn_gemm_opts* o, hipStream_t st, int phase) {
  PRN_REQUIRE(o != nullptr && w && x && y && images_ws && (splits == 1 || partial), "prn_split_conv_taps: null operand");
  PRN_REQUIRE(o->split_kind == PRN_PIECES_F16 && (C & 31) == 0 && KH > 0 && KW > 0, "prn_split_conv_taps: fp16 pieces and C %% 32 == 0 only");
  const int K = KH * KW * C, HW = Ho * Wo;
  const int mtiles = cdiv(M, 128), kslices = K / 32, ptiles = cdiv(HW, 128);
  PRN_REQUIRE((int64_t)kslices * IMG_U4 * 16 < (1LL << 31) && (int64_t)C * XH * XW < (1LL << 29) && (int64_t)M * HW < (1LL << 29),
              "prn_split_conv_taps: operand larger than a buffer descriptor");
  if (phase != 2) {
    if (int e = cut_weight(w, images_ws, M, K, 1, (long long)M * K, PRN_PIECES_F16, st, "prn_split_conv_taps/prepare", KH * KW)) return e;
    Split16Args a;
    a.img = (const uint4*)images_ws; a.ex = (const int*)((const char*)images_ws + (int64_t)mtiles * kslices * IMG16_U4 * 16);
    a.x = x; a.bias = bias; a.addend = addend; a.y = y; a.partial = partial;
    a.M = M; a.K = K; a.B = B; a.HW = HW; a.epi = epi; a.mtiles = mtiles; a.kslices = kslices; a.ptiles = ptiles;
    a.total = mtiles * ptiles * B; a.splits = splits; a.zx = 0; a.zy = 0; a.slice = (long long)B * M * HW;
    a.C = C; a.XH = XH; a.XW = XW; a.Wo = Wo; a.KW = KW; a.stride = stride; a.pad = pad;
    auto al16 = [](const void* q) { return (reinterpret_cast<uintptr_t>(q) & 15) == 0; };
    a.wide = (HW & 3) == 0 && ((int64_t)M * HW & 3) == 0 && al16(y) && al16(addend) && al16(partial);
    a.store_policy = 1;
    if (o->split_products >= 4) hipLaunchKernelGGL((split16_gemm_kernel<4, 1>), dim3(a.total, splits), dim3(256), 0, st, a);
    else hipLaunchKernelGGL((split16_gemm_kernel<3, 1>), dim3(a.total, splits), dim3(256), 0, st, a);
    PRN_CHECK_LAUNCH("prn_split_conv_taps");
  }
  if (splits > 1 && phase != 1) return prn_launch_reduce_epilogue(partial, bias, addend, y, (int64_t)B * M * HW, M, HW, splits, epi, st);
  return 0;
}

int prn_split_conv_up2(const float* wp, const float* x, const float* bias, float* y, void* images_ws, int M, int C, int B, int H, int W, int epi, const prn_gemm_opts* o,
                       hipStream_t st) {
  PRN_REQUIRE(o != nullptr && wp && x && y && images_ws, "prn_split_conv_up2: null operand");
  PRN_REQUIRE(o->split_kind == PRN_PIECES_F16 && (C & 31) == 0 && (W & 3) == 0 && (reinterpret_cast<uintptr_t>(y) & 15) == 0, "prn_split_conv_up2: fp16 pieces, C %% 32 == 0, W %% 4 == 0");
  const int K = 4 * C, HW = H * W;
  const int mtiles = cdiv(M, 128), kslices = K / 32, ptiles = cdiv(HW, 128);
  PRN_REQUIRE((int64_t)kslices * IMG_U4 * 16 < (1LL << 31) && (int64_t)C * HW < (1LL << 29) && (int64_t)B * M * HW * 4 < (1LL << 31), "prn_split_conv_up2: operand too large");
  if (int e = cut_weight(wp, images_ws, M, K, 4, (long long)M * K, PRN_PIECES_F16, st, "prn_split_conv_up2/prepare", 4)) return e;
  Split16Args a;
  a.img = (const uint4*)images_ws; a.ex = (const int*)((const char*)images_ws + (int64_t)4 * mtiles * kslices * IMG16_U4 * 16);
  a.x = x; a.bias = bias; a.addend = nullptr; a.y = y; a.partial = nullptr;
  a.M = M; a.K = K; a.B = B; a.HW = HW; a.epi = epi; a.mtiles = mtiles; a.kslices = kslices; a.ptiles = ptiles;
  a.total = mtiles * ptiles * B * 4; a.splits = 1; a.zx = 0; a.zy = 0; a.slice = 0;
  a.C = C; a.XH = H; a.XW = W; a.Wo = W; a.KW = 2; a.stride = 1; a.pad = 0;
  a.wide = 1; a.store_policy = 1;
  if (o->split_products >= 4) hipLaunchKernelGGL((split16_gemm_kernel<4, 2>), dim3(a.total, 1), dim3(256), 0, st, a);
  else hipLaunchKernelGGL((split16_gemm_kernel<3, 2>), dim3(a.total, 1), dim3(256), 0, st, a);
  PRN_CHECK_LAUNCH("prn_split_conv_up2");
  return 0;
}
```

### planerecnet_amd/ops.py

```python
import ctypes

import os
import threading
import weakref

import torch

from . import _lib, profiling
from ._lib import ConvDesc, GemmOpts, IN_ZERO, IN_REFLECT, IN_UP2_REFLECT, IN_DILATED, IN_UP2_PHASE, IN_EMBED1, EPI_NONE, EPI_RELU, EPI_SIGMOID, lib, check


_SIDE = {}
WGRAD_ASYNC = bool(int(os.environ.get("PRN_WGRAD_ASYNC", "0")))


WGRAD_WGS_ASYNC = os.environ.get("PRN_WGRAD_WGS_ASYNC", "512")


_POLICY = {"split_mode": int(os.environ.get("PRN_SPLIT_GEMM", "1")),
           "kind": _lib.PIECES_BF16 if os.environ.get("PRN_SPLIT_KIND", "f16") == "bf16" else _lib.PIECES_F16,
           "products": int(os.environ.get("PRN_SPLIT16_PRODUCTS", "3")),
           "min_gflop": float(os.environ.get("PRN_SPLIT_MIN_GFLOP", "4.0")),
           "min_tiles": int(os.environ.get("PRN_SPLIT_MIN_TILES", os.environ.get("PRN_SPLIT_MIN_TILES_EVAL", "300"))),
           "wgrad_wgs": int(os.environ.get("PRN_WGRAD_WGS", "0") or 0),
# ... 310 lines not shown
    side = getattr(_TLS, "side", None)
    return ctypes.c_void_p(side if side is not None else _raw_stream(_cur_dev()))


def _p(t):
    return None if t is None else ctypes.c_void_p(t.data_ptr())


def _ptr(t):
    return None if t is None else t.data_ptr()


OPERAND_EPOCH = [0]


def _dev(*ts):
    for t in ts:
        if t is not None and (not t.is_cuda or t.dtype != torch.float32):
            raise RuntimeError("planerecnet_amd ops need fp32 tensors resident on the MI355X (got %s %s); "
                               "there is no CPU fallback" % (t.device, t.dtype))


def _c(t):
    return t if (t is None or t.is_contiguous()) else t.contiguous()


_DESC = {}


def _desc(B, C, H, W, M, K, stride, pad, Ho, Wo, mode=IN_ZERO, dil=1, epi=EPI_NONE, ystride=0, yH=0, yW=0):
    oe = _opts_entry("conv1x1" in SPLIT_SKIP)
    key = (B, C, H, W, M, K, stride, pad, Ho, Wo, mode, dil, epi, ystride, yH, yW, oe[2])
    e = _DESC.get(key)
    if e is None:
        d = ConvDesc(B, C, H, W, M, K, K, stride, pad, Ho, Wo, mode, dil, epi, ystride, yH, yW, 0, oe[0])
        ref = ctypes.byref(d)
        fb = lib.prn_conv2d_fwd_ws_bytes(ref)
        wb = lib.prn_conv2d_wgrad_ws_bytes(ref) if (mode != IN_DILATED and K != 4 and ystride <= 1) else 0
        if fb < 0 or wb < 0:
            raise RuntimeError(lib.prn_last_error().decode())
        d.kind = lib.prn_conv2d_kernel_kind(ref)
        off = ctypes.c_int64(0)
        parts = lib.prn_conv2d_fwd_partials(ref, ctypes.byref(off)) if ystride <= 1 else 0
        e = _DESC[key] = (d, ref, fb, wb, (parts, off.value // 4) if parts > 1 else None)
    return e




def _out_hw(H, W, K, stride, pad, mode):
    if mode == IN_REFLECT:
        return H, W
    if mode == IN_UP2_REFLECT:
        return 2 * H, 2 * W
    return (H + 2 * pad - K) // stride + 1, (W + 2 * pad - K) // stride + 1


FUSED_SPLIT_SUM = os.environ.get("PRN_CONV_FUSED_REDUCE", "0") == "1"
_COUNTERS = {}
TILE_COUNTERS = 4096


def _counters(dev):
    key = (dev.index, torch._C._cuda_getCurrentRawStream(dev.index))
    c = _COUNTERS.get(key)
    if c is None:
        c = _COUNTERS[key] = torch.zeros(TILE_COUNTERS, device=dev, dtype=torch.int32)
    return c


def split_products():
    return float(max(_POLICY["products"], 3)) if _POLICY["kind"] == _lib.PIECES_F16 else 6.0


def _gemm_family(M, K, B, HW, nz, flops):
    if gemm_pipe(M, K, B, HW, nz) >= 1:
        return "split_gemm_kernel", split_products() * flops, flops
    return "conv_igemm_kernel", flops, flops



SPLIT_CACHE = os.environ.get("PRN_SPLIT_CACHE", "auto")
SPLIT_CACHE_MIN_TILES = int(os.environ.get("PRN_SPLIT_CACHE_MIN_TILES", "2500"))
_SPLIT_IMG = {}
_STAMP = {}
_STAMP_GEN = [0]
_SPLIT_ITEMS = [None, None, 0]
_PIPE = {}
SPLIT_STATS = {"hits": 0, "cuts": 0, "uncached": 0, "refreshes": 0}


_SPLIT_POLICY = {"train": int(os.environ.get("PRN_SPLIT_MIN_TILES", os.environ.get("PRN_SPLIT_MIN_TILES_TRAIN", "300"))),
                 "eval": int(os.environ.get("PRN_SPLIT_MIN_TILES", os.environ.get("PRN_SPLIT_MIN_TILES_EVAL", "300")))}
_SPLIT_POLICY["current"] = _POLICY["min_tiles"]


def split_gemm_policy(which):
    n = _SPLIT_POLICY[which]
    _SPLIT_POLICY["mode"] = which
    if _SPLIT_POLICY.get("current") != n:
        _SPLIT_POLICY["current"] = n
        _POLICY["min_tiles"] = n


def autotune_split_policy(run_step, which, alternatives=None, steps=10, skip=3, rounds=2, margin=0.015, reduce_max=None):
    import time
    base = _SPLIT_POLICY[which]
    alts = [a for a in (alternatives if alternatives is not None else ((300,) if which == "train" else (10 ** 9,))) if a != base]
    if _POLICY["split_mode"] != 1 or "PRN_SPLIT_MIN_TILES" in os.environ or not alts:
        return {"tuned": False, "min_tiles": base}
    times = {n: [] for n in [base] + alts}
    for _ in range(rounds):
        for n in [base] + alts:
            _SPLIT_POLICY[which] = n
            for _ in range(skip):
                run_step()
            torch.cuda.synchronize()
            t0 = time.perf_counter()
            for _ in range(steps):
                run_step()
            torch.cuda.synchronize()
            times[n].append((time.perf_counter() - t0) / steps)
    if reduce_max is not None:
        flat = reduce_max([t for n in [base] + alts for t in times[n]])
        for i, n in enumerate([base] + alts):
            times[n] = flat[i * rounds:(i + 1) * rounds]
    best = base
    for n in alts:
        if max(times[n]) < (1.0 - margin) * min(times[best]):
            best = n
    _SPLIT_POLICY[which] = best
    return {"tuned": True, "min_tiles": best, "default": base, "ms_per_step": {str(n): [round(1e3 * t, 2) for t in v] for n, v in times.items()}}


def gemm_pipe(M, K, B, HW, nz):
    oe = _opts_entry()
    key = (M, K, B, HW, nz, oe[2])
    v = _PIPE.get(key)
    if v is None:
        v = _PIPE[key] = lib.prn_gemm_pipe(int(M), int(K), int(B), int(HW), int(nz), oe[1])
    return v


class _SplitEntry:
    __slots__ = ("owner", "tensor", "stamp", "images", "dims", "ptr")


def _stamp(t):
    p = t.data_ptr()
    _STAMP_GEN[0] += 1
    _STAMP[p] = (_STAMP_GEN[0], weakref.ref(t))


def _stamp_of(ptr):
    s = _STAMP.get(ptr)
    if s is None:
        return None
    if s[1]() is None:
        _STAMP.pop(ptr, None)
        return None
    return s[0]


def _split_drop(ptr, stamp=True):
    if stamp:
        _STAMP.pop(ptr, None)
    if _SPLIT_IMG.pop(ptr, None) is not None:
        _SPLIT_ITEMS[0] = None
        OPERAND_EPOCH[0] += 1


def _split_state(e):
    if e.owner is not None:
        o = e.owner()
        if o is None or o.data_ptr() != e.ptr:
            return None
        return o._version
    return _stamp_of(e.ptr)


def _prep_items(entries, dev):
    import numpy as np
    items = np.zeros(len(entries), dtype=np.dtype([("src", "u8"), ("dst", "u8"), ("M", "i4"), ("K", "i4"), ("nz", "i4"), ("pad", "i4"), ("zw", "i8"), ("first", "i8")]))
    blocks = rblocks = 0
    for i, e in enumerate(entries):
        M, K, nz, _ = e.dims
        items[i] = (e.ptr, e.images.data_ptr(), M, K, nz, 0, rblocks, blocks)
        blocks += (nz * ((M + 127) // 128) * ((K + 31) // 32) * 512 + 255) // 256
        rblocks += (nz * ((M + 127) // 128) * 128 + 3) // 4
    return torch.from_numpy(items.view(np.uint8).reshape(-1).copy()).to(dev), blocks, rblocks


def split_images(t, M, K, nz, cols=None):
    training = _SPLIT_POLICY.get("mode", "eval") == "train"
    if SPLIT_CACHE in ("0", False) or (SPLIT_CACHE == "eval" and training):
        return None
    floor = SPLIT_CACHE_MIN_TILES if (SPLIT_CACHE == "eval" or (SPLIT_CACHE == "auto" and not training)) else 0
    if cols is not None and ((M + 127) // 128) * ((cols[1] + 127) // 128) * cols[0] * nz < floor:
        if t.data_ptr() in _SPLIT_IMG:
            _split_drop(t.data_ptr(), stamp=False)
        return None
    kind = _POLICY["kind"]
    ptr = t.data_ptr()
    e = _SPLIT_IMG.get(ptr)
    if e is not None:
        cur = _split_state(e)
        if cur is not None and cur == e.stamp and e.dims == (M, K, nz, kind):
            SPLIT_STATS["hits"] += 1
            return _p(e.images)
        if cur is None or e.dims != (M, K, nz, kind):
            _split_drop(ptr, stamp=False)
            e = None
    if e is None:
        owner = t if isinstance(t, torch.nn.Parameter) else (t._base if isinstance(t._base, torch.nn.Parameter) else None)
        if owner is None and _stamp_of(ptr) is None:
            SPLIT_STATS["uncached"] += 1
            return None
        if owner is not None and owner.data_ptr() != ptr:
            return None
        e = _SplitEntry()
        e.owner = weakref.ref(owner) if owner is not None else None
        e.tensor = None if owner is not None else t
        e.ptr, e.dims = ptr, (M, K, nz, kind)
        nb = lib.prn_split_images_bytes(M, K, nz)
        e.images = torch.empty(nb, device=t.device, dtype=torch.uint8)
        _SPLIT_IMG[ptr] = e
        _SPLIT_ITEMS[0] = None
        OPERAND_EPOCH[0] += 1
        if owner is not None:
            weakref.finalize(owner, lambda p=ptr, r=e: _split_drop(p) if _SPLIT_IMG.get(p) is r else None)
    check(lib.prn_split_prepare(ctypes.c_void_p(ptr), _p(e.images), M, K, nz, kind, _stream()), "prn_split_prepare")
    e.stamp = _split_state(e)
    SPLIT_STATS["cuts"] += 1
    if os.environ.get("PRN_SPLIT_DEBUG"):
        SPLIT_STATS.setdefault("who", {}).setdefault((M, K, nz, "param" if e.owner is not None else "derived"), []).append(SPLIT_STATS["refreshes"])
    return _p(e.images)


def split_images_ptr(t, M, K, nz, cols=None):
    r = split_images(t, M, K, nz, cols)
    return None if r is None else r.value


def split_refresh_all():
    if SPLIT_CACHE == "eval" or SPLIT_CACHE in ("0", False):
        return
    if _SPLIT_POLICY.get("mode", "eval") != "train":
        return
    dead = [p for p, e in _SPLIT_IMG.items() if _split_state(e) is None]
    for p in dead:
        _split_drop(p)
    if not _SPLIT_IMG:
        return
    kind = _POLICY["kind"]
    for e in [e for e in _SPLIT_IMG.values() if e.dims[3] != kind]:
        _split_drop(e.ptr, stamp=False)
    entries = list(_SPLIT_IMG.values())
    if not entries:
        return
    if _SPLIT_ITEMS[0] is None or _SPLIT_ITEMS[1] != [id(e) for e in entries]:
        items, blocks, rblocks = _prep_items(entries, entries[0].images.device)
        _SPLIT_ITEMS[0], _SPLIT_ITEMS[1], _SPLIT_ITEMS[2] = items, [id(e) for e in entries], (blocks, rblocks)
    check(lib.prn_split_prepare_batched(_p(_SPLIT_ITEMS[0]), len(entries), _SPLIT_ITEMS[2][0], _SPLIT_ITEMS[2][1], kind, _stream()), "prn_split_prepare_batched")
    for e in entries:
        e.stamp = _split_state(e)
    SPLIT_STATS["refreshes"] += 1


def conv_fwd_raw(x, w2d, bias, addend, M, K, stride, pad, Ho, Wo, mode=IN_ZERO, dil=1, epi=EPI_NONE, scatter2=None):
    B, C, H, W = x.shape
    if scatter2 is None:
        y = torch.empty(B, M, Ho, Wo, device=x.device, dtype=torch.float32)
        d_, ref, nbytes, _, _ = _desc(B, C, H, W, M, K, stride, pad, Ho, Wo, mode, dil, epi)
        wimg = split_images(w2d, M, C, 1, (B, Ho * Wo)) if (d_.kind >= 2 and K == 1 and stride == 1) else None
    else:
        wimg = None
        y = torch.zeros(B, M, scatter2[0], scatter2[1], device=x.device, dtype=torch.float32)
        _, ref, nbytes, _, _ = _desc(B, C, H, W, M, K, stride, pad, Ho, Wo, mode, dil, epi, 2, scatter2[0], scatter2[1])
    ws = torch.empty(nbytes // 4, device=x.device, dtype=torch.float32) if nbytes else None
    cnt = _counters(x.device) if (nbytes and FUSED_SPLIT_SUM) else None
    if profiling._enabled:
        kind = lib.prn_conv2d_kernel_kind(ref)
        direct = kind == 1
        split = kind >= 2
        nb_ = 4.0 * (x.numel() + w2d.numel() + y.numel() + (addend.numel() if addend is not None else 0))
        fl = 2.0 * M * C * K * K * B * Ho * Wo / (dil * dil)
        with profiling.span("conv3x3_direct" if direct else ("split_gemm_kernel" if split else "conv_igemm_kernel"), "hbm" if direct else "mfma",
                            nb_ if direct else (split_products() * fl if split else fl), ref=None if direct else fl, nbytes=nb_,
                            tag=None if direct else ("conv", C, H, W, M, K, stride, mode, dil, B)):
            check(lib.prn_conv2d_fwd_counted(ref, _p(x), _p(w2d), wimg, _p(bias), _p(addend), _p(y), _p(ws), _p(cnt), _stream(), 1), "prn_conv2d_fwd")
        if nbytes and kind != 2:
            with profiling.span("reduce_epilogue_kernel", "hbm", float(nbytes) + 4.0 * y.numel()):
                check(lib.prn_conv2d_fwd_counted(ref, _p(x), _p(w2d), wimg, _p(bias), _p(addend), _p(y), _p(ws), _p(cnt), _stream(), 2), "prn_conv2d_fwd")
    else:
        check(lib.prn_conv2d_fwd_counted(ref, _p(x), _p(w2d), wimg, _p(bias), _p(addend), _p(y), _p(ws), _p(cnt), _stream(), 0), "prn_conv2d_fwd")
    return y


def conv_wgrad_raw(x, dy, M, K, stride, pad, mode):
    B, C, H, W = x.shape
    if mode == IN_UP2_PHASE:
        Ho, Wo = 2 * H, 2 * W
        dw = torch.empty(4, M, C, 2, 2, device=x.device, dtype=torch.float32)
    else:
        Ho, Wo = dy.shape[2:]
        dw = torch.empty(M, C, K, K, device=x.device, dtype=torch.float32)
    _, ref, _, nbytes, _ = _desc(B, C, H, W, M, K, stride, pad, Ho, Wo, mode)
    ws = _wspace(nbytes, x.device)
    if profiling._enabled:
        wkind = lib.prn_conv2d_wgrad_kernel_kind(ref, 1)
        direct = wkind == 1
        fl_w = 2.0 * M * C * K * K * B * Ho * Wo
        with profiling.span("conv3x3_direct" if direct else ("wgrad16_kernel" if wkind == 2 else "conv_wgrad_kernel"), "hbm" if direct else "mfma",
                            4.0 * (x.numel() + dy.numel()) if direct else (split_products() * fl_w if wkind == 2 else fl_w), ref=None if direct else fl_w,
                            nbytes=4.0 * (x.numel() + dy.numel() + dw.numel()),
                            tag=None if direct else ("wgrad", C, H, W, M, K, stride, mode, 1, B)):
            check(lib.prn_conv2d_wgrad_phase(ref, _p(x), _p(dy), _p(dw), _p(ws), _stream(), 1), "prn_conv2d_wgrad")
        if nbytes:
            with profiling.span("reduce_splits_kernel", "hbm", float(nbytes) + 4.0 * dw.numel()):
                check(lib.prn_conv2d_wgrad_phase(ref, _p(x), _p(dy), _p(dw), _p(ws), _stream(), 2), "prn_conv2d_wgrad")
    else:
        check(lib.prn_conv2d_wgrad(ref, _p(x), _p(dy), _p(dw), _p(ws), _stream()), "prn_conv2d_wgrad")
    return dw


WGRAD_GROUP_MAX = 16


def conv_wgrad_grouped_raw(xs, dys, M, K, stride, pad, mode):
    G = len(xs)
    B, C, H, W = xs[0].shape
    Ho, Wo = dys[0].shape[2:]
    dev = xs[0].device
    _, ref, _, _, _ = _desc(B, C, H, W, M, K, stride, pad, Ho, Wo, mode)
    nbytes = lib.prn_conv2d_wgrad_grouped_ws_bytes(ref, G)
    if nbytes < 0:
        raise RuntimeError(lib.prn_last_error().decode())
    dw = torch.empty(G, M, C, K, K, device=dev, dtype=torch.float32)
    ws = _wspace(nbytes, dev)
    px = (ctypes.c_void_p * G)(*[t.data_ptr() for t in xs])
    pdy = (ctypes.c_void_p * G)(*[t.data_ptr() for t in dys])
    check(lib.prn_conv2d_wgrad_grouped(ref, G, px, pdy, _p(dw), _p(ws), _stream()), "prn_conv2d_wgrad_grouped")
    return dw


_FLIP_USED = set()


def flip_transpose(w):
    _FLIP_USED.add(w.data_ptr())
    e = _FLIPPED.get(w.data_ptr())
    if e is not None and tuple(t._version for t in e[0]) == e[1] and e[2].shape[1] == w.shape[0]:
        return e[2]
    M, C, KH, KW = w.shape
    wt = torch.empty(C, M, KH, KW, device=w.device, dtype=torch.float32)
    check(lib.prn_weight_flip_transpose(_p(w), _p(wt), M, C, KH, KW, _stream()), "prn_weight_flip_transpose")
    return wt
# ... 245 lines not shown
        dp = conv_fwd_raw(dy, wt, None, None, C, K, 1, 2, Hv + 2, Wv + 2)
        dx = torch.empty(B, C, H, W, device=dy.device, dtype=torch.float32)
        check(lib.prn_pad_fold(_p(dp), _p(dx), B, C, H, W, 1 if mode == IN_UP2_REFLECT else 0, _stream()), "prn_pad_fold")
        return dx if addend is None else dx + addend
    if stride == 1:
        return conv_fwd_raw(dy, wt, None, addend, C, K, 1, K - 1 - pad, H, W)
    if stride != 2:
        raise RuntimeError("conv dgrad: stride %d not implemented" % stride)
    if K == 1 and pad == 0 and addend is None:
        return conv_fwd_raw(dy, wt, None, None, C, 1, 1, 0, dy.shape[2], dy.shape[3], scatter2=(H, W))
    if K == 1 and pad == 0:
        return conv_fwd_raw(dy, wt, None, None, C, 1, 1, 0, dy.shape[2], dy.shape[3], scatter2=(H, W)) + addend
    return conv_fwd_raw(dy, wt, None, addend, C, K, 1, K - 1 - pad, H, W, IN_DILATED, 2)


class _Conv2d(torch.autograd.Function):
    @staticmethod
    def forward(ctx, x, w, bias, addend, stride, pad, mode, epi, fork=False):
        _dev(x, w, bias, addend)
        x0, bias_param = x, bias
        x, w, bias, addend = _c(x), _c(w), _c(bias), _c(addend)
        M, C, K, _ = w.shape
        assert x.shape[1] == C, (x.shape, w.shape)
        Ho, Wo = _out_hw(x.shape[2], x.shape[3], K, stride, pad, mode)
        ctx.wino_v = None
        if winograd_ok(x.shape[0], C, x.shape[2], x.shape[3], M, K, stride, pad, mode, epi):
            keep = [] if (WINOGRAD_WGRAD and ctx.needs_input_grad[1]) else None
            y = conv3x3_winograd_raw(x, winograd_weights(w)[0], bias, addend, M, mode, epi, keep)
            if keep:
                ctx.wino_v = keep[0]
        else:
            y = conv_fwd_raw(x, w, bias, addend, M, K, stride, pad, Ho, Wo, mode, 1, epi)
        ctx.save_for_backward(x, w, y if epi != EPI_NONE else None)
        ctx.cfg = (stride, pad, mode, epi, bias is not None, addend is not None)
        ctx.bias = bias_param
        ctx.fork = fork
        if fork:
            ctx.set_materialize_grads(False)
            return y, x0
        return y

    @staticmethod
    def backward(ctx, dy, dfork=None):
        x, w, y = ctx.saved_tensors
        stride, pad, mode, epi, has_bias, has_add = ctx.cfg
        if dy is None:
            return (dfork,) + (None,) * 8
        dy = _c(dy)
        dfork = _c(dfork)
        if epi == EPI_RELU:
            dy = torch.ops.aten.threshold_backward(dy, y, 0.0)
        elif epi == EPI_SIGMOID:
            dy = dy * y * (1 - y)
        M, C, K, _ = w.shape
        if WINOGRAD_WGRAD and winograd_ok(x.shape[0], C, x.shape[2], x.shape[3], M, K, stride, pad, mode, EPI_NONE):
            V, ctx.wino_v = ctx.wino_v, None

            def wgrad():
                return conv3x3_winograd_wgrad_raw(x, dy, M, mode, V)
        else:
            V = None

            def wgrad():
                return conv_wgrad_raw(x, dy, M, K, stride, pad, mode)
        if _defer(ctx.needs_input_grad[1], w):
            gkey = None
            if V is None and K in (1, 3, 7) and mode in (IN_ZERO, IN_REFLECT) and M > 2 and dy.shape[0] * dy.shape[2] * dy.shape[3] <= WGRAD_GROUP_PIXELS:
                gkey = ("conv", tuple(x.shape), tuple(dy.shape[2:]), M, K, stride, pad, mode)
            _deferred_wgrad(w, (x, dy) if V is None else (x, dy, V), wgrad, gkey, fast=True)
            dx = conv_dgrad_raw(dy, w, x.shape, stride, pad, mode, dfork) if ctx.needs_input_grad[0] else None
            dfork = None
            dw = None
        else:
            dx = conv_dgrad_raw(dy, w, x.shape, stride, pad, mode, dfork) if ctx.needs_input_grad[0] else None
            dfork = None
            dw = wgrad() if ctx.needs_input_grad[1] else None
        if dfork is not None and dx is not None:
            dx = dx + dfork
        db = _bias_grad(has_bias and ctx.needs_input_grad[2], ctx.bias, dy)
        da = dy if (has_add and ctx.needs_input_grad[3]) else None
        return dx, dw, db, da, None, None, None, None, None


class _ConvUp2(torch.autograd.Function):

    @staticmethod
    def forward(ctx, x, w, bias):
        _dev(x, w, bias)
        bias_param = bias
        x, w, bias = _c(x), _c(w), _c(bias)
        B, C, H, W = x.shape
        M = w.shape[0]
        assert w.shape[1:] == (C, 3, 3), (x.shape, w.shape)
        wp = torch.empty(4, M, C, 2, 2, device=x.device, dtype=torch.float32)
        check(lib.prn_up2_phase_weights(_p(w), _p(wp), M, C, _stream()), "prn_up2_phase_weights")
        y = conv_fwd_raw(x, wp, bias, None, M, 2, 1, 0, 2 * H, 2 * W, IN_UP2_PHASE)
        ctx.save_for_backward(x, w)
        ctx.has_bias = bias is not None
        ctx.bias = bias_param
        return y

    @staticmethod
    def backward(ctx, dy):
        x, w = ctx.saved_tensors
        dy = _c(dy)
        B, C, H, W = x.shape
        M = w.shape[0]
        dx = dw = db = None
        if ctx.needs_input_grad[0]:
            kd = torch.empty(C, M, 4, 4, device=x.device, dtype=torch.float32)
            check(lib.prn_up2_dgrad_weights(_p(w), _p(kd), M, C, _stream()), "prn_up2_dgrad_weights")
            dp = conv_fwd_raw(dy, kd, None, None, C, 4, 2, 3, H + 2, W + 2)
            dx = torch.empty_like(x)
            check(lib.prn_replicate_fold(_p(dp), _p(dx), B, C, H, W, _stream()), "prn_replicate_fold")
        def wgrad():
            dyp = torch.empty(4, B, M, H, W, device=x.device, dtype=torch.float32)
            check(lib.prn_space_to_depth2(_p(dy), _p(dyp), B, M, H, W, _stream()), "prn_space_to_depth2")
            dwp = conv_wgrad_raw(x, dyp, M, 2, 1, 0, IN_UP2_PHASE)
            dwo = torch.empty_like(w)
            check(lib.prn_up2_wgrad_combine(_p(dwp), _p(dwo), M, C, _stream()), "prn_up2_wgrad_combine")
            if getattr(_TLS, "side", None) is not None:
                _HELD.append((dyp, dwp))
            return dwo
        if _defer(ctx.needs_input_grad[1], w):
            _deferred_wgrad(w, (x, dy), wgrad, fast=True)
        elif ctx.needs_input_grad[1]:
            dw = wgrad()
        db = _bias_grad(ctx.has_bias and ctx.needs_input_grad[2], ctx.bias, dy)
        return dx, dw, db


UP2_SUBPIXEL = bool(int(os.environ.get("PRN_UP2_SUBPIXEL", "1")))


def conv2d(x, w, bias=None, stride=1, pad=0, in_mode=IN_ZERO, epilogue=EPI_NONE, addend=None):
    if in_mode == IN_UP2_REFLECT and UP2_SUBPIXEL and epilogue == EPI_NONE and addend is None and x.shape[2] > 1 and x.shape[3] > 1:
        return _ConvUp2.apply(x, w, bias)
    return _Conv2d.apply(x, w, bias, addend, stride, pad, in_mode, epilogue, False)


_UP2_PHASE = {}


def conv_up2_inference(x, w, bias=None, relu=False):
    _dev(x, w, bias)
    x, w, bias = _c(x), _c(w), _c(bias)
    B, C, H, W = x.shape
    M = w.shape[0]
    assert w.shape[1:] == (C, 3, 3), (x.shape, w.shape)
    if not (UP2_SUBPIXEL and H > 1 and W > 1):
        return conv2d(x, w, bias, 1, 1, IN_UP2_REFLECT, EPI_RELU if relu else EPI_NONE)
    e = _UP2_PHASE.get(w.data_ptr())
    if e is None or e[0]() is not w or e[1] != w._version:
        wp = torch.empty(4, M, C, 2, 2, device=x.device, dtype=torch.float32)
        check(lib.prn_up2_phase_weights(_p(w), _p(wp), M, C, _stream()), "prn_up2_phase_weights")
        ptr = w.data_ptr()
        e = _UP2_PHASE[ptr] = (weakref.ref(w), w._version, wp)
        weakref.finalize(w, lambda p=ptr, r=e[0]: _UP2_PHASE.pop(p, None) if (_UP2_PHASE.get(p) or (None,))[0] is r else None)
    return conv_fwd_raw(x, e[2], bias, None, M, 2, 1, 0, 2 * H, 2 * W, IN_UP2_PHASE, 1, EPI_RELU if relu else EPI_NONE)


def conv2d_fork(x, w, bias=None, stride=1, pad=0, in_mode=IN_ZERO, epilogue=EPI_NONE, addend=None):
    return _Conv2d.apply(x, w, bias, addend, stride, pad, in_mode, epilogue, True)


_DCN = {}


def _dcn_desc(B, C, H, W, M, stride, pad, raw, max_offset, epi=EPI_NONE):
    oe = _opts_entry("colgrad" in SPLIT_SKIP)
    key = (B, C, H, W, M, stride, pad, raw, float(max_offset), epi, oe[2])
    e = _DCN.get(key)
    if e is None:
        Ho, Wo = (H + 2 * pad - 3) // stride + 1, (W + 2 * pad - 3) // stride + 1
        d = _lib.DcnDesc(B, C, H, W, M, stride, pad, Ho, Wo, int(raw), float(max_offset), epi, oe[0])
        ref = ctypes.byref(d)
        sizes = [lib.prn_dcnv2_table_bytes(ref), lib.prn_dcnv2_fwd_ws_bytes(ref), lib.prn_dcnv2_bwd_weight_ws_bytes(ref), lib.prn_dcnv2_bwd_ws_bytes(ref)]
        if min(sizes) < 0:
            raise RuntimeError(lib.prn_last_error().decode())
        e = _DCN[key] = (d, ref, sizes[0], sizes[1], sizes[2], sizes[3])
    return e


def _f32(nbytes, dev):
    return torch.empty(max(nbytes // 4, 1), device=dev, dtype=torch.float32)


def dcn_table(x_shape, M, offset, mask, stride, pad, raw, max_offset):
    B, C, H, W = x_shape
    _, ref, tb, _, _, _ = _dcn_desc(B, C, H, W, M, stride, pad, raw, max_offset)
    table = _f32(tb, offset.device)
    check(lib.prn_dcnv2_table(ref, _p(offset), _p(mask), _p(table), _stream()), "prn_dcnv2_table")
    return table

# ... 678 lines not shown
```

### planerecnet_amd/planerecnet.py

```python
import os

import torch
import torch.nn as nn
import torch.nn.functional as F

from . import ops, timer
from .backbone import can_fold, construct_backbone, conv_bn, folded_bn
from .config import cfg
from .fpn import FPN
from .funcs import bias_init_with_prob
from .nms import mask_nms, matrix_nms


_COORD = {}


def _coord_channels(feat):
    B, _, h, w = feat.shape
    key = (B, h, w, feat.device)
    c = _COORD.get(key)
    if c is None:
        xr = torch.linspace(-1, 1, w, device=feat.device)
        yr = torch.linspace(-1, 1, h, device=feat.device)
        y, x = torch.meshgrid(yr, xr, indexing="ij")
# ... 1 lines not shown
    return c


def _coord_channels_resized(feat, size):
    B, _, h, w = feat.shape
    key = (B, h, w, feat.device, int(size[0]), int(size[1]))
    c = _COORD.get(key)
    if c is None:
        with torch.no_grad():
            c = _COORD[key] = ops.resize_bilinear(_coord_channels(feat), size).contiguous()
    return c


def _conv_gn_relu(x, conv, gn):
    return ops.group_norm_relu(ops.conv2d(x, conv.weight, conv.bias, pad=conv.padding[0]), gn.weight, gn.bias, gn.num_groups, gn.eps)


class PlaneRecNet(nn.Module):
    def __init__(self, cfg):
        super().__init__()
        self.device = torch.device(cfg.device)
        self.depth_decoder_indices = cfg.depth.selected_layers
        self.fpn_indices = cfg.fpn.selected_layers
        s = cfg.solov2
        self.num_classes, self.num_kernels, self.num_grids = cfg.num_classes, s.num_kernels, s.num_grids
        self.instance_in_features, self.instance_strides = s.instance_in_features, s.fpn_instance_strides
        self.instance_in_channels, self.instance_channels = cfg.fpn.num_features, s.instance_channels
        self.mask_in_features, self.mask_in_channels = s.masks_in_features, cfg.fpn.num_features
        self.mask_channels, self.num_masks = s.masks_channels, s.num_masks
        self.max_before_nms, self.score_threshold, self.update_threshold = s.nms_pre, s.score_thr, s.update_thr
        self.mask_threshold, self.max_per_img = s.mask_thr, s.top_k
        self.nms_kernel, self.nms_sigma, self.nms_type = s.nms_kernel, s.nms_sigma, s.nms_type

        self.backbone = construct_backbone(cfg.backbone)
        if cfg.freeze_bn:
            self.freeze_bn()
        src = self.backbone.channels
        self.fpn = FPN([src[i] for i in self.fpn_indices], start_level=cfg.fpn.start_level)
        self.depth_decoder = DepthDecoder_FPN()
        self.inst_head = SOLOv2InsHead(cfg, [cfg.fpn.num_features] * len(s.instance_in_features))
        self.mask_head = SOLOv2MaskHead(cfg, [cfg.fpn.num_features] * len(s.masks_in_features))

    def _refresh_dgrad_weights(self):
        fw = self.__dict__.get("_flipped")
        if fw is not None and any(m._merged()[0] is not d for m, d in self.__dict__.get("_flip_dcn", ())):
            for d in fw.data:
                ops._FLIPPED.pop(d.data_ptr(), None)
            fw = None
        if fw is None:
            from .dcn import DeformableConv2d
            dcns = [m for m in self.modules() if isinstance(m, DeformableConv2d)]
            dcn_w = {id(m.regular_conv.weight) for m in dcns}
            dcn_om = {id(c.weight) for m in dcns for c in (m.offset_conv, m.modulator_conv)}
            items = []
            for m in self.modules():
                if isinstance(m, nn.Conv2d) and m.weight.requires_grad and m.weight.is_cuda and id(m.weight) not in dcn_om:
                    M, C, KH, KW = m.weight.shape
                    items.append((m.weight, (M, C * KH * KW, 1, 1) if id(m.weight) in dcn_w else (M, C, KH, KW)))
            for m in dcns:
                if m.offset_conv.weight.requires_grad and m.offset_conv.weight.is_cuda:
                    w27 = m._merged()[0]
                    items.append((m.offset_conv.weight, tuple(w27.shape), w27, (m.modulator_conv.weight,)))
            self.__dict__["_flip_dcn"] = [(m, e[2]) for m, e in zip([m for m in dcns if m.offset_conv.weight.requires_grad and m.offset_conv.weight.is_cuda],
                                                                     [e for e in items if len(e) > 2])]
            fw = self.__dict__["_flipped"] = ops.FlippedWeights(items)
            self.__dict__["_flip_steps"] = 0
        self.__dict__["_flip_steps"] += 1
        if self.__dict__["_flip_steps"] == 3:
            used = [(w, shp, d, gd[1:]) for (w, shp), d, gd in zip(fw.weights, fw.data, fw.guards) if d.data_ptr() in ops._FLIP_USED]
            if used and len(used) < len(fw.weights):
                for d in fw.data:
                    ops._FLIPPED.pop(d.data_ptr(), None)
                fw = self.__dict__["_flipped"] = ops.FlippedWeights(used)
        fw.refresh()
        mine = self.__dict__.get("_param_ids")
        if mine is None:
            mine = self.__dict__["_param_ids"] = {id(p) for p in self.parameters()}
        seen = [w for w in ops.winograd_seen() if id(w) in mine]
        ww = self.__dict__.get("_wino")
        if seen and (ww is None or len(ww.weights) != len(seen)):
            ww = self.__dict__["_wino"] = ops.WinogradWeights(seen)
        if ww is not None:
            ww.refresh()
        ops.split_refresh_all()
        ops.vouch_refreshed([t for gd in fw.guards for t in gd])
        if ww is not None:
            ops.vouch_refreshed(ww.weights)

    def forward(self, x):
        if x.is_cuda:
            ops.split_gemm_policy("train" if self.training else "eval")
        if self.training and torch.is_grad_enabled() and x.is_cuda:
            self._refresh_dgrad_weights()
        with timer.env("backbone"):
            enc = self.backbone(x)
        with timer.env("fpn"):
            feats, fenc = self.fpn([enc[i] for i in self.fpn_indices], return_inputs=True)
            enc = list(enc)
            for i, f in zip(self.fpn_indices, fenc):
                enc[i] = f
        with timer.env("instance head"):
            ins_feats, feats[0] = self.split_feats([feats[f] for f in range(len(self.instance_in_features))], fork=True)
            cate_pred, kernel_pred = self.inst_head(ins_feats)
        with timer.env("mask head"):
            mask_pred = self.mask_head([feats[f] for f in range(len(self.mask_in_features))])
        with timer.env("depth_decoder"):
            depth_pred = self.depth_decoder([enc[i] for i in self.depth_decoder_indices], mask_pred, kernel_pred)
        with timer.env("Inferencing"):
            if self.training:
                return mask_pred, cate_pred, kernel_pred, depth_pred
            from .metrics import category_scores
            return self.inference(mask_pred, category_scores(cate_pred), kernel_pred, depth_pred, x)

    @staticmethod
    def split_feats(feats, fork=False):
        h, w = feats[0].shape[2:]
        if fork:
            r, f0 = ops.resize_bilinear_fork(feats[0], (int(h * 0.5), int(w * 0.5)))
            return (r, feats[1], feats[2], feats[3]), f0
        return (ops.resize_bilinear(feats[0], (int(h * 0.5), int(w * 0.5))), feats[1], feats[2], feats[3])

    def _flush_bn_counters(self):
        for m in self.modules():
            if isinstance(m, nn.BatchNorm2d):
                ops.flush_batch_count(m)

    def state_dict(self, *args, **kwargs):
        self._flush_bn_counters()
        return super().state_dict(*args, **kwargs)

    def load_state_dict(self, *args, **kwargs):
        for m in self.modules():
            m.__dict__.pop("_prn_nbt_pending", None)
        return super().load_state_dict(*args, **kwargs)

    def save_weights(self, path):
        torch.save(self.state_dict(), path)

    def load_weights(self, path):
        self.load_state_dict(torch.load(path, map_location="cpu"))

    def init_weights(self, backbone_path):
        self.backbone.init_backbone(backbone_path)
        self.init_head_weights()

    def init_head_weights(self):
        for name, module in self.named_modules():
            if isinstance(module, nn.Conv2d) and module not in self.backbone.backbone_modules:
                nn.init.xavier_uniform_(module.weight.data)
                if module.bias is not None:
                    if "inst_head" in name and "cate_pred" in name:
                        module.bias.data.fill_(bias_init_with_prob(cfg.solov2.focal_loss_init_pi))
                    else:
                        module.bias.data.fill_(0)

    def freeze_bn(self, enable=False):
        for module in self.modules():
            if isinstance(module, nn.BatchNorm2d):
                module.train() if enable else module.eval()
                module.weight.requires_grad = enable
                module.bias.requires_grad = enable

    def inference(self, pred_masks, pred_cates, pred_kernels, pred_depths, batched_images, ori_size=None):
        from .metrics import mask_boxes, mask_stats
        assert torch.is_tensor(pred_cates) or len(pred_cates) == len(pred_kernels)
        B = pred_masks.shape[0]
# ... 315 lines not shown
```

Measured before the change: 192.3.

## Cache fp16-split weight images for tap-walked strided and up2 convolutions

Adds a taps-aware split-weight preparation entry point and lets the tap-walked and sub-pixel (up2) split convolution paths consume precomputed weight images instead of re-cutting weights into fp16 pieces on every call. Up2 phase and dgrad derived weights are kept persistently per parameter and refreshed only when the parameter version changes. Strided downsample 1x1 convolutions in bottleneck blocks now also use cached images. The aim is to remove per-call weight-cut kernels and allocations. In exchange the cache keying and invalidation logic becomes more complex and uses more memory.

```diff
diff --git a/include/prn.h b/include/prn.h
--- a/include/prn.h
+++ b/include/prn.h
@@ -49,6 +49,7 @@
 int prn_gemm_pipe(int M, int K, int B, int HW, int nz, const prn_gemm_opts* opts);
 int64_t prn_split_images_bytes(int M, int K, int nz);
 int prn_split_prepare(const float* w, void* images, int M, int K, int nz, int kind, void* stream);
+int prn_split_prepare_taps(const float* w, void* images, int M, int K, int nz, int taps, void* stream);
 int prn_split_prepare_batched(const void* items_dev, int n_items, int64_t total_blocks, int64_t total_row_blocks, int kind, void* stream);
 int prn_conv2d_fwd(const prn_conv_desc* d, const float* x, const float* w, const float* bias,
                    const float* addend, float* y, void* ws, void* stream);
diff --git a/planerecnet_amd/_lib.py b/planerecnet_amd/_lib.py
--- a/planerecnet_amd/_lib.py
+++ b/planerecnet_amd/_lib.py
@@ -63,6 +63,7 @@
     "prn_gemm_pipe": (c_int, [c_int, c_int, c_int, c_int, c_int, _OP]),
     "prn_split_images_bytes": (c_i64, [c_int, c_int, c_int]),
     "prn_split_prepare": (c_int, [P, P, c_int, c_int, c_int, c_int, P]),
+    "prn_split_prepare_taps": (c_int, [P, P, c_int, c_int, c_int, c_int, P]),
     "prn_split_prepare_batched": (c_int, [P, c_int, c_i64, c_i64, c_int, P]),
     "prn_conv2d_fwd": (c_int, [_DP, P, P, P, P, P, P, P]),
     "prn_conv2d_fwd_ragged": (c_int, [_DP, P, P, P, P, P, P, P]),
diff --git a/planerecnet_amd/blocks.py b/planerecnet_amd/blocks.py
--- a/planerecnet_amd/blocks.py
+++ b/planerecnet_amd/blocks.py
@@ -174,7 +174,7 @@
         wd = blk.downsample[0].weight
         wdt = derived(ops.flip_transpose(wd))
         p.wd, p.wd_t = ptr(wd), ptr(wdt)
-        p.wd_img = images(wd, Q, C, 1, (B, Ho * Wo), info[I_WD_IMG])
+        p.wd_img = images(wd, Q, C, 1, (B, Ho * Wo), info[I_WD_IMG] and (st.stride == 1 or ops.TAP_IMAGES))
         p.wd_t_img = images(wdt, C, Q, 1, (B, H * W), info[I_WDT_IMG])
     p.w2 = p.b2 = p.w2_t = p.u2 = p.ut2 = p.u2_img = p.ut2_img = p.w27 = p.b27 = p.w27_t = p.w2_cols_t = p.w2_cols_t_img = None
     if st.conv2 == CONV2_DCN:
diff --git a/planerecnet_amd/csrc/prn_bottleneck.hip b/planerecnet_amd/csrc/prn_bottleneck.hip
--- a/planerecnet_amd/csrc/prn_bottleneck.hip
+++ b/planerecnet_amd/csrc/prn_bottleneck.hip
@@ -180,7 +180,7 @@
   out[PRN_BLK_BN_GRAD_FLOATS] = L->q_bn;
   out[PRN_BLK_HANDOVERS] = L->lazy1 | (L->v1 << 1) | (L->lazy2 << 2) | (L->lazy3g << 3) | (L->v2g << 4) | (L->lazy2g << 5);
   out[PRN_BLK_NEEDS_W1_IMG] = prn_conv2d_kernel_kind(&L->c1) >= 2; out[PRN_BLK_NEEDS_W3_IMG] = prn_conv2d_kernel_kind(&L->c3) >= 2;
-  out[PRN_BLK_NEEDS_WD_IMG] = (L->d.downsample && L->d.stride == 1 && prn_conv2d_kernel_kind(&L->cd) >= 2) ? 1 : 0;
+  out[PRN_BLK_NEEDS_WD_IMG] = (L->d.downsample && prn_conv2d_kernel_kind(&L->cd) >= 2) ? 1 : 0;
   out[PRN_BLK_NEEDS_W1T_IMG] = prn_conv2d_kernel_kind(&L->g1) >= 2; out[PRN_BLK_NEEDS_W3T_IMG] = prn_conv2d_kernel_kind(&L->g3) >= 2;
   out[PRN_BLK_NEEDS_WDT_IMG] = (L->d.downsample && L->d.stride == 1 && prn_conv2d_kernel_kind(&L->gd) >= 2) ? 1 : 0;
   out[PRN_BLK_NEEDS_U_IMG] = (L->conv2_path == PRN_BLK_CONV2_WINOGRAD && prn_gemm_pipe(L->d.planes, L->d.planes, 1, L->P4, 36, &L->d.opts) >= 1) ? 1 : 0;
@@ -242,7 +242,7 @@
   if (d.downsample) {
     float* cd = f32(save, L.s_cd);
     float* rd = f32(ws, L.f_res);
-    PRN_TRY(prn_conv2d_fwd_counted(&L.cd, x, p->wd, d.stride == 1 ? p->wd_img : nullptr, nullptr, nullptr, cd, raw(ws, L.f_cd, L.f_res - L.f_cd), nullptr, stream, 0));
+    PRN_TRY(prn_conv2d_fwd_counted(&L.cd, x, p->wd, p->wd_img, nullptr, nullptr, cd, raw(ws, L.f_cd, L.f_res - L.f_cd), nullptr, stream, 0));
     PRN_TRY(prn_bn_train_fwd(cd, std_, p->gamma[3], p->beta[3], nullptr, rd, p->running_mean[3], p->running_var[3], L.small2 ? nullptr : bnws, B, Q, Ho * Wo, d.eps[3],
                              d.momentum[3], 0, stream));
     res = rd;
diff --git a/planerecnet_amd/csrc/prn_common.h b/planerecnet_amd/csrc/prn_common.h
--- a/planerecnet_amd/csrc/prn_common.h
+++ b/planerecnet_amd/csrc/prn_common.h
@@ -122,9 +122,9 @@
 int64_t prn_split_gemm_partial_bytes(int M, int B, int HW, int nz, int splits);
 int prn_split_gemm(const float* w, const void* w_images, const float* x, const float* bias, const float* addend, float* y, void* images_ws, float* partial, int M,
                    int K, int B, int HW, int nz, int64_t zw, int64_t zx, int64_t zy, int epi, int splits, const prn_gemm_opts* opts, hipStream_t st, int phase);
-int prn_split_conv_taps(const float* w, const float* x, const float* bias, const float* addend, float* y, void* images_ws, float* partial, int M, int C, int B, int XH,
+int prn_split_conv_taps(const float* w, const void* w_images, const float* x, const float* bias, const float* addend, float* y, void* images_ws, float* partial, int M, int C, int B, int XH,
                         int XW, int Ho, int Wo, int KH, int KW, int stride, int pad, int epi, int splits, const prn_gemm_opts* o, hipStream_t st, int phase);
-int prn_split_conv_up2(const float* wp, const float* x, const float* bias, float* y, void* images_ws, int M, int C, int B, int H, int W, int epi, const prn_gemm_opts* o,
+int prn_split_conv_up2(const float* wp, const void* w_images, const float* x, const float* bias, float* y, void* images_ws, int M, int C, int B, int H, int W, int epi, const prn_gemm_opts* o,
                        hipStream_t st);
 static inline prn_gemm_opts prn_opts_or_zero(const prn_gemm_opts* o) {
   prn_gemm_opts z;
diff --git a/planerecnet_amd/csrc/prn_conv.hip b/planerecnet_amd/csrc/prn_conv.hip
--- a/planerecnet_amd/csrc/prn_conv.hip
+++ b/planerecnet_amd/csrc/prn_conv.hip
@@ -1544,11 +1544,11 @@
     }
     if (up2_plan_of(d) && addend == nullptr && (reinterpret_cast<uintptr_t>(y) & 15) == 0) {
       if (phase == 2) return 0;
-      return prn_split_conv_up2(w, x, bias, y, ws, d->M, d->C, d->B, d->H, d->W, d->epilogue, &d->opts, (hipStream_t)stream);
+      return prn_split_conv_up2(w, w_images, x, bias, y, ws, d->M, d->C, d->B, d->H, d->W, d->epilogue, &d->opts, (hipStream_t)stream);
     }
     if (const int st = taps_plan_of(d)) {
       const int64_t ib = (prn_split_gemm_image_bytes(d->M, d->C * d->KH * d->KW, 1) + 255) & ~255LL;
-      return prn_split_conv_taps(w, x, bias, addend, y, ws, (float*)((char*)ws + ib), d->M, d->C, d->B, d->H, d->W, d->Ho, d->Wo, d->KH, d->KW, d->stride, d->pad, d->epilogue,
+      return prn_split_conv_taps(w, w_images, x, bias, addend, y, ws, (float*)((char*)ws + ib), d->M, d->C, d->B, d->H, d->W, d->Ho, d->Wo, d->KH, d->KW, d->stride, d->pad, d->epilogue,
                                  st, &d->opts, (hipStream_t)stream, phase);
     }
   }
diff --git a/planerecnet_amd/csrc/prn_gemm_split.hip b/planerecnet_amd/csrc/prn_gemm_split.hip
--- a/planerecnet_amd/csrc/prn_gemm_split.hip
+++ b/planerecnet_amd/csrc/prn_gemm_split.hip
@@ -201,6 +201,15 @@
   if (lane == 0) ex[row] = mx > 0.f ? __builtin_amdgcn_frexp_expf(mx) : 0;
 }
 
+__device__ __forceinline__ void cut16_load8(const float* __restrict__ wrow, bool row_ok, int K, int k0, int sh, int taps, float (&v)[8]) {
+  const int C = K / (taps > 1 ? taps : 1);
+#pragma unroll
+  for (int j = 0; j < 8; ++j) {
+    const int kp = k0 + j;
+    const int ksrc = taps > 1 ? (kp % C) * taps + kp / C : kp;
+    v[j] = (row_ok && kp < K) ? ldexpf(wrow[ksrc], sh) : 0.f;
+  }
+}
 __global__ void split16_prepare_kernel(const float* __restrict__ w, uint4* __restrict__ img, const int* __restrict__ ex, int M, int K, long long zw, int mtiles, int kslices,
                                        long long total, int taps = 1) {
   const long long i = (long long)blockIdx.x * 256 + threadIdx.x;
@@ -210,13 +219,7 @@
   const int m = mt * 128 + r, k0 = ks * 32 + g * 8;
   const int sh = 14 - ex[z * (mtiles * 128) + m];
   float v[8];
-  const int C = K / taps;
-#pragma unroll
-  for (int j = 0; j < 8; ++j) {
-    const int kp = k0 + j;
-    const int ksrc = taps > 1 ? (kp % C) * taps + kp / C : kp;
-    v[j] = (m < M && kp < K) ? ldexpf(w[z * zw + (long long)m * K + ksrc], sh) : 0.f;
-  }
+  cut16_load8(w + z * zw + (long long)m * K, m < M, K, k0, sh, taps, v);
   uint4 h, l;
   split2_f16(v[0], v[1], h.x, l.x); split2_f16(v[2], v[3], h.y, l.y); split2_f16(v[4], v[5], h.z, l.z); split2_f16(v[6], v[7], h.w, l.w);
   uint4* o = img + t * IMG16_U4;
@@ -478,7 +481,7 @@
   }
 }
 
-struct PrepItem { const float* src; uint4* dst; int M, K, nz, pad; long long zw; long long first; };
+struct PrepItem { const float* src; uint4* dst; int M, K, nz, taps; long long zw; long long first; };
 __global__ void split_prepare_batched_kernel(const PrepItem* __restrict__ items, int n) {
   int lo = 0, hi = n - 1;
   const long long blk = blockIdx.x;
@@ -542,13 +545,12 @@
   const int sh = 14 - ex[z * (mtiles * 128) + m];
   float v[8];
   const float* wr = it.src + z * (long long)it.M * it.K + (long long)m * it.K + k0;
-  if (m < it.M && k0 + 8 <= it.K && (it.K & 3) == 0 && (reinterpret_cast<uintptr_t>(it.src) & 15) == 0) {
+  if (it.taps <= 1 && m < it.M && k0 + 8 <= it.K && (it.K & 3) == 0 && (reinterpret_cast<uintptr_t>(it.src) & 15) == 0) {
     const float4 a = *reinterpret_cast<const float4*>(wr), b = *reinterpret_cast<const float4*>(wr + 4);
     v[0] = ldexpf(a.x, sh); v[1] = ldexpf(a.y, sh); v[2] = ldexpf(a.z, sh); v[3] = ldexpf(a.w, sh);
     v[4] = ldexpf(b.x, sh); v[5] = ldexpf(b.y, sh); v[6] = ldexpf(b.z, sh); v[7] = ldexpf(b.w, sh);
   } else {
-#pragma unroll
-    for (int j = 0; j < 8; ++j) v[j] = (m < it.M && k0 + j < it.K) ? ldexpf(wr[j], sh) : 0.f;
+    cut16_load8(wr - k0, m < it.M, it.K, k0, sh, it.taps, v);
   }
   uint4 h, l;
   split2_f16(v[0], v[1], h.x, l.x); split2_f16(v[2], v[3], h.y, l.y); split2_f16(v[4], v[5], h.z, l.z); split2_f16(v[6], v[7], h.w, l.w);
@@ -623,6 +625,10 @@
   PRN_REQUIRE(w && images && M > 0 && K > 0 && nz > 0 && (reinterpret_cast<uintptr_t>(images) & 15) == 0, "prn_split_prepare: bad arguments");
   PRN_REQUIRE(kind == PRN_PIECES_F16 || kind == PRN_PIECES_BF16, "prn_split_prepare: kind is PRN_PIECES_F16 or PRN_PIECES_BF16");
   return cut_weight(w, images, M, K, nz, (long long)M * K, kind, (hipStream_t)stream, "prn_split_prepare");
+}
+extern "C" int prn_split_prepare_taps(const float* w, void* images, int M, int K, int nz, int taps, void* stream) {
+  PRN_REQUIRE(w && images && M > 0 && K > 0 && nz > 0 && taps > 0 && K % taps == 0 && (reinterpret_cast<uintptr_t>(images) & 15) == 0, "prn_split_prepare_taps: bad arguments");
+  return cut_weight(w, images, M, K, nz, (long long)M * K, PRN_PIECES_F16, (hipStream_t)stream, "prn_split_prepare_taps", taps);
 }
 extern "C" int prn_gemm_pipe(int M, int K, int B, int HW, int nz, const prn_gemm_opts* opts) {
   return prn_split_gemm_plan(M, K, B, HW, nz, opts);
@@ -682,18 +688,23 @@
   return 0;
 }
 
-int prn_split_conv_taps(const float* w, const float* x, const float* bias, const float* addend, float* y, void* images_ws, float* partial, int M, int C, int B, int XH,
+int prn_split_conv_taps(const float* w, const void* w_images, const float* x, const float* bias, const float* addend, float* y, void* images_ws, float* partial, int M, int C, int B, int XH,
                         int XW, int Ho, int Wo, int KH, int KW, int stride, int pad, int epi, int splits, const prn_gemm_opts* o, hipStream_t st, int phase) {
-  PRN_REQUIRE(o != nullptr && w && x && y && images_ws && (splits == 1 || partial), "prn_split_conv_taps: null operand");
+  PRN_REQUIRE(o != nullptr && w && x && y && (w_images || images_ws) && (splits == 1 || partial), "prn_split_conv_taps: null operand");
   PRN_REQUIRE(o->split_kind == PRN_PIECES_F16 && (C & 31) == 0 && KH > 0 && KW > 0, "prn_split_conv_taps: fp16 pieces and C %% 32 == 0 only");
   const int K = KH * KW * C, HW = Ho * Wo;
   const int mtiles = cdiv(M, 128), kslices = K / 32, ptiles = cdiv(HW, 128);
   PRN_REQUIRE((int64_t)kslices * IMG_U4 * 16 < (1LL << 31) && (int64_t)C * XH * XW < (1LL << 29) && (int64_t)M * HW < (1LL << 29),
               "prn_split_conv_taps: operand larger than a buffer descriptor");
   if (phase != 2) {
-    if (int e = cut_weight(w, images_ws, M, K, 1, (long long)M * K, PRN_PIECES_F16, st, "prn_split_conv_taps/prepare", KH * KW)) return e;
+    const void* images = w_images;
+    if (images == nullptr) {
+      if (int e = cut_weight(w, images_ws, M, K, 1, (long long)M * K, PRN_PIECES_F16, st, "prn_split_conv_taps/prepare", KH * KW)) return e;
+      images = images_ws;
+    }
+    PRN_REQUIRE((reinterpret_cast<uintptr_t>(images) & 15) == 0, "prn_split_conv_taps: images must be 16-byte aligned");
     Split16Args a;
-    a.img = (const uint4*)images_ws; a.ex = (const int*)((const char*)images_ws + (int64_t)mtiles * kslices * IMG16_U4 * 16);
+    a.img = (const uint4*)images; a.ex = (const int*)((const char*)images + (int64_t)mtiles * kslices * IMG16_U4 * 16);
     a.x = x; a.bias = bias; a.addend = addend; a.y = y; a.partial = partial;
     a.M = M; a.K = K; a.B = B; a.HW = HW; a.epi = epi; a.mtiles = mtiles; a.kslices = kslices; a.ptiles = ptiles;
     a.total = mtiles * ptiles * B; a.splits = splits; a.zx = 0; a.zy = 0; a.slice = (long long)B * M * HW;
@@ -709,16 +720,21 @@
   return 0;
 }
 
-int prn_split_conv_up2(const float* wp, const float* x, const float* bias, float* y, void* images_ws, int M, int C, int B, int H, int W, int epi, const prn_gemm_opts* o,
+int prn_split_conv_up2(const float* wp, const void* w_images, const float* x, const float* bias, float* y, void* images_ws, int M, int C, int B, int H, int W, int epi, const prn_gemm_opts* o,
                        hipStream_t st) {
-  PRN_REQUIRE(o != nullptr && wp && x && y && images_ws, "prn_split_conv_up2: null operand");
+  PRN_REQUIRE(o != nullptr && wp && x && y && (w_images || images_ws), "prn_split_conv_up2: null operand");
   PRN_REQUIRE(o->split_kind == PRN_PIECES_F16 && (C & 31) == 0 && (W & 3) == 0 && (reinterpret_cast<uintptr_t>(y) & 15) == 0, "prn_split_conv_up2: fp16 pieces, C %% 32 == 0, W %% 4 == 0");
   const int K = 4 * C, HW = H * W;
   const int mtiles = cdiv(M, 128), kslices = K / 32, ptiles = cdiv(HW, 128);
   PRN_REQUIRE((int64_t)kslices * IMG_U4 * 16 < (1LL << 31) && (int64_t)C * HW < (1LL << 29) && (int64_t)B * M * HW * 4 < (1LL << 31), "prn_split_conv_up2: operand too large");
-  if (int e = cut_weight(wp, images_ws, M, K, 4, (long long)M * K, PRN_PIECES_F16, st, "prn_split_conv_up2/prepare", 4)) return e;
+  const void* images = w_images;
+  if (images == nullptr) {
+    if (int e = cut_weight(wp, images_ws, M, K, 4, (long long)M * K, PRN_PIECES_F16, st, "prn_split_conv_up2/prepare", 4)) return e;
+    images = images_ws;
+  }
+  PRN_REQUIRE((reinterpret_cast<uintptr_t>(images) & 15) == 0, "prn_split_conv_up2: images must be 16-byte aligned");
   Split16Args a;
-  a.img = (const uint4*)images_ws; a.ex = (const int*)((const char*)images_ws + (int64_t)4 * mtiles * kslices * IMG16_U4 * 16);
+  a.img = (const uint4*)images; a.ex = (const int*)((const char*)images + (int64_t)4 * mtiles * kslices * IMG16_U4 * 16);
   a.x = x; a.bias = bias; a.addend = nullptr; a.y = y; a.partial = nullptr;
   a.M = M; a.K = K; a.B = B; a.HW = HW; a.epi = epi; a.mtiles = mtiles; a.kslices = kslices; a.ptiles = ptiles;
   a.total = mtiles * ptiles * B * 4; a.splits = 1; a.zx = 0; a.zy = 0; a.slice = 0;
diff --git a/planerecnet_amd/ops.py b/planerecnet_amd/ops.py
--- a/planerecnet_amd/ops.py
+++ b/planerecnet_amd/ops.py
@@ -416,7 +416,9 @@
 
 SPLIT_CACHE = os.environ.get("PRN_SPLIT_CACHE", "auto")
 SPLIT_CACHE_MIN_TILES = int(os.environ.get("PRN_SPLIT_CACHE_MIN_TILES", "2500"))
+TAP_IMAGES = bool(int(os.environ.get("PRN_TAP_IMAGES", "1")))
 _SPLIT_IMG = {}
+_SPLIT_TAPS = set()
 _STAMP = {}
 _STAMP_GEN = [0]
 _SPLIT_ITEMS = [None, None, 0]
@@ -477,7 +479,7 @@
 
 
 class _SplitEntry:
-    __slots__ = ("owner", "tensor", "stamp", "images", "dims", "ptr")
+    __slots__ = ("owner", "tensor", "stamp", "images", "dims", "ptr", "taps")
 
 
 def _stamp(t):
@@ -496,12 +498,13 @@
     return s[0]
 
 
-def _split_drop(ptr, stamp=True):
+def _split_drop(ptr, stamp=True, taps=None):
     if stamp:
         _STAMP.pop(ptr, None)
-    if _SPLIT_IMG.pop(ptr, None) is not None:
-        _SPLIT_ITEMS[0] = None
-        OPERAND_EPOCH[0] += 1
+    for key in ([ptr] + [(ptr, t) for t in _SPLIT_TAPS]) if taps is None else [ptr if taps <= 1 else (ptr, taps)]:
+        if _SPLIT_IMG.pop(key, None) is not None:
+            _SPLIT_ITEMS[0] = None
+            OPERAND_EPOCH[0] += 1
 
 
 def _split_state(e):
@@ -519,31 +522,35 @@
     blocks = rblocks = 0
     for i, e in enumerate(entries):
         M, K, nz, _ = e.dims
-        items[i] = (e.ptr, e.images.data_ptr(), M, K, nz, 0, rblocks, blocks)
+        items[i] = (e.ptr, e.images.data_ptr(), M, K, nz, e.taps, rblocks, blocks)
         blocks += (nz * ((M + 127) // 128) * ((K + 31) // 32) * 512 + 255) // 256
         rblocks += (nz * ((M + 127) // 128) * 128 + 3) // 4
     return torch.from_numpy(items.view(np.uint8).reshape(-1).copy()).to(dev), blocks, rblocks
 
 
-def split_images(t, M, K, nz, cols=None):
+def split_images(t, M, K, nz, cols=None, taps=1):
     training = _SPLIT_POLICY.get("mode", "eval") == "train"
     if SPLIT_CACHE in ("0", False) or (SPLIT_CACHE == "eval" and training):
         return None
     floor = SPLIT_CACHE_MIN_TILES if (SPLIT_CACHE == "eval" or (SPLIT_CACHE == "auto" and not training)) else 0
+    ptr = t.data_ptr()
+    key = ptr if taps <= 1 else (ptr, taps)
+    assert taps >= 1 and K % taps == 0, (K, taps)
     if cols is not None and ((M + 127) // 128) * ((cols[1] + 127) // 128) * cols[0] * nz < floor:
-        if t.data_ptr() in _SPLIT_IMG:
-            _split_drop(t.data_ptr(), stamp=False)
+        if key in _SPLIT_IMG:
+            _split_drop(ptr, stamp=False, taps=taps)
         return None
     kind = _POLICY["kind"]
-    ptr = t.data_ptr()
-    e = _SPLIT_IMG.get(ptr)
+    if taps > 1 and kind != _lib.PIECES_F16:
+        return None
+    e = _SPLIT_IMG.get(key)
     if e is not None:
         cur = _split_state(e)
         if cur is not None and cur == e.stamp and e.dims == (M, K, nz, kind):
             SPLIT_STATS["hits"] += 1
             return _p(e.images)
         if cur is None or e.dims != (M, K, nz, kind):
-            _split_drop(ptr, stamp=False)
+            _split_drop(ptr, stamp=False, taps=taps)
             e = None
     if e is None:
         owner = t if isinstance(t, torch.nn.Parameter) else (t._base if isinstance(t._base, torch.nn.Parameter) else None)
@@ -555,19 +562,24 @@
         e = _SplitEntry()
         e.owner = weakref.ref(owner) if owner is not None else None
         e.tensor = None if owner is not None else t
-        e.ptr, e.dims = ptr, (M, K, nz, kind)
+        e.ptr, e.dims, e.taps = ptr, (M, K, nz, kind), max(int(taps), 1)
         nb = lib.prn_split_images_bytes(M, K, nz)
         e.images = torch.empty(nb, device=t.device, dtype=torch.uint8)
-        _SPLIT_IMG[ptr] = e
+        _SPLIT_IMG[key] = e
+        if taps > 1:
+            _SPLIT_TAPS.add(taps)
         _SPLIT_ITEMS[0] = None
         OPERAND_EPOCH[0] += 1
         if owner is not None:
-            weakref.finalize(owner, lambda p=ptr, r=e: _split_drop(p) if _SPLIT_IMG.get(p) is r else None)
-    check(lib.prn_split_prepare(ctypes.c_void_p(ptr), _p(e.images), M, K, nz, kind, _stream()), "prn_split_prepare")
+            weakref.finalize(owner, lambda p=ptr, k=key, r=e, tp=taps: _split_drop(p, taps=tp) if _SPLIT_IMG.get(k) is r else None)
+    if taps > 1:
+        check(lib.prn_split_prepare_taps(ctypes.c_void_p(ptr), _p(e.images), M, K, nz, taps, _stream()), "prn_split_prepare_taps")
+    else:
+        check(lib.prn_split_prepare(ctypes.c_void_p(ptr), _p(e.images), M, K, nz, kind, _stream()), "prn_split_prepare")
     e.stamp = _split_state(e)
     SPLIT_STATS["cuts"] += 1
     if os.environ.get("PRN_SPLIT_DEBUG"):
-        SPLIT_STATS.setdefault("who", {}).setdefault((M, K, nz, "param" if e.owner is not None else "derived"), []).append(SPLIT_STATS["refreshes"])
+        SPLIT_STATS.setdefault("who", {}).setdefault((M, K, nz, "param" if e.owner is not None else "derived") + ((taps,) if taps > 1 else ()), []).append(SPLIT_STATS["refreshes"])
     return _p(e.images)
 
 
@@ -581,9 +593,9 @@
         return
     if _SPLIT_POLICY.get("mode", "eval") != "train":
         return
-    dead = [p for p, e in _SPLIT_IMG.items() if _split_state(e) is None]
-    for p in dead:
-        _split_drop(p)
+    dead = [e for e in _SPLIT_IMG.values() if _split_state(e) is None]
+    for e in dead:
+        _split_drop(e.ptr)
     if not _SPLIT_IMG:
         return
     kind = _POLICY["kind"]
@@ -606,7 +618,14 @@
     if scatter2 is None:
         y = torch.empty(B, M, Ho, Wo, device=x.device, dtype=torch.float32)
         d_, ref, nbytes, _, _ = _desc(B, C, H, W, M, K, stride, pad, Ho, Wo, mode, dil, epi)
-        wimg = split_images(w2d, M, C, 1, (B, Ho * Wo)) if (d_.kind >= 2 and K == 1 and stride == 1) else None
+        wimg = None
+        if d_.kind >= 2 and K == 1 and stride == 1:
+            wimg = split_images(w2d, M, C, 1, (B, Ho * Wo))
+        elif d_.kind >= 2 and TAP_IMAGES and w2d.is_contiguous():
+            if mode == IN_UP2_PHASE:
+                wimg = split_images(w2d, M, 4 * C, 4, (B, H * W), taps=4) if (K == 2 and addend is None) else None
+            elif mode == IN_ZERO and stride == 2 and K in (1, 4):
+                wimg = split_images(w2d, M, C * K * K, 1, (B, Ho * Wo), taps=K * K)
     else:
         wimg = None
         y = torch.zeros(B, M, scatter2[0], scatter2[1], device=x.device, dtype=torch.float32)
@@ -1018,6 +1037,61 @@
         return dx, dw, db, da, None, None, None, None, None
 
 
+_UP2_TRAIN = {}
+
+
+def _up2_derive(w, which, M, C):
+    check((lib.prn_up2_phase_weights if which == "wp" else lib.prn_up2_dgrad_weights)(_p(w), _p(_UP2_TRAIN[w.data_ptr()][1][which][0]), M, C, _stream()),
+          "prn_up2_phase_weights" if which == "wp" else "prn_up2_dgrad_weights")
+
+
+def _up2_operand(w, which):
+    M, C = w.shape[:2]
+    shape = (4, M, C, 2, 2) if which == "wp" else (C, M, 4, 4)
+    known = _UP2_TRAIN.get(w.data_ptr())
+    if known is not None and known[0]() is not None and known[0]() is not w and known[0]().data_ptr() == w.data_ptr() and known[0]().shape == w.shape:
+        w = known[0]()
+    if not (TAP_IMAGES and isinstance(w, torch.nn.Parameter)):
+        t = torch.empty(shape, device=w.device, dtype=torch.float32)
+        check((lib.prn_up2_phase_weights if which == "wp" else lib.prn_up2_dgrad_weights)(_p(w), _p(t), M, C, _stream()),
+              "prn_up2_phase_weights" if which == "wp" else "prn_up2_dgrad_weights")
+        return t
+    ptr = w.data_ptr()
+    e = _UP2_TRAIN.get(ptr)
+    if e is None or e[0]() is not w:
+        if e is not None:
+            _up2_pop(ptr)
+        e = _UP2_TRAIN[ptr] = [weakref.ref(w), {}]
+        weakref.finalize(w, lambda p=ptr, r=e[0]: _up2_pop(p) if (_UP2_TRAIN.get(p) or (None,))[0] is r else None)
+    b = e[1].get(which)
+    if b is None:
+        b = e[1][which] = [torch.empty(shape, device=w.device, dtype=torch.float32), None]
+    if b[1] != w._version:
+        _up2_derive(w, which, M, C)
+        b[1] = w._version
+        _stamp(b[0])
+    return b[0]
+
+
+def _up2_pop(ptr):
+    e = _UP2_TRAIN.pop(ptr, None)
+    for b in (e[1].values() if e is not None else ()):
+        _split_drop(b[0].data_ptr())
+
+
+def up2_refresh_all():
+    for ptr, e in list(_UP2_TRAIN.items()):
+        w = e[0]()
+        if w is None or w.data_ptr() != ptr:
+            _up2_pop(ptr)
+            continue
+        for which, b in e[1].items():
+            if b[1] != w._version:
+                _up2_derive(w, which, w.shape[0], w.shape[1])
+                b[1] = w._version
+                _stamp(b[0])
+
+
 class _ConvUp2(torch.autograd.Function):
 
     @staticmethod
@@ -1028,8 +1102,7 @@
         B, C, H, W = x.shape
         M = w.shape[0]
         assert w.shape[1:] == (C, 3, 3), (x.shape, w.shape)
-        wp = torch.empty(4, M, C, 2, 2, device=x.device, dtype=torch.float32)
-        check(lib.prn_up2_phase_weights(_p(w), _p(wp), M, C, _stream()), "prn_up2_phase_weights")
+        wp = _up2_operand(w, "wp")
         y = conv_fwd_raw(x, wp, bias, None, M, 2, 1, 0, 2 * H, 2 * W, IN_UP2_PHASE)
         ctx.save_for_backward(x, w)
         ctx.has_bias = bias is not None
@@ -1044,8 +1117,7 @@
         M = w.shape[0]
         dx = dw = db = None
         if ctx.needs_input_grad[0]:
-            kd = torch.empty(C, M, 4, 4, device=x.device, dtype=torch.float32)
-            check(lib.prn_up2_dgrad_weights(_p(w), _p(kd), M, C, _stream()), "prn_up2_dgrad_weights")
+            kd = _up2_operand(w, "kd")
             dp = conv_fwd_raw(dy, kd, None, None, C, 4, 2, 3, H + 2, W + 2)
             dx = torch.empty_like(x)
             check(lib.prn_replicate_fold(_p(dp), _p(dx), B, C, H, W, _stream()), "prn_replicate_fold")
diff --git a/planerecnet_amd/planerecnet.py b/planerecnet_amd/planerecnet.py
--- a/planerecnet_amd/planerecnet.py
+++ b/planerecnet_amd/planerecnet.py
@@ -107,6 +107,7 @@
             ww = self.__dict__["_wino"] = ops.WinogradWeights(seen)
         if ww is not None:
             ww.refresh()
+        ops.up2_refresh_all()
         ops.split_refresh_all()
         ops.vouch_refreshed([t for gd in fw.guards for t in gd])
         if ww is not None:
```

After: 192.7 (median of 6 runs). Within noise of the previous version (+0.2%).
